# JuliaRobotics/RigidBodyDynamics.jl

Hardware: AMD Instinct MI355X
Metric: ABA dynamics! evals/sec (Atlas 30-DoF, batch) (higher is better)
Workload: dtype f64

## Files before the change

### rigidbodydynamics.jl_amd/csrc/rbd_bank.hpp

```cpp
#pragma once

#ifndef RBD_BANK_WAVES
#define RBD_BANK_WAVES 2
#endif
#ifndef RBD_BANK_FK_LDS
#define RBD_BANK_FK_LDS 0
#endif
#ifndef RBD_BANK_HANDOFF_LDS
#define RBD_BANK_HANDOFF_LDS 0
#endif

#ifdef RBD_BANK_FIXED_NL
#define RBD_BANK_UNROLL _Pragma("unroll")
namespace rbd { constexpr int kBankNs[] = {RBD_BANK_FIXED_NS}; }
#define RBD_BK_NL RBD_BANK_FIXED_NL
#define RBD_BK_L0 RBD_BANK_FIXED_L0
#define RBD_BK_NS(l) kBankNs[l]
#ifdef RBD_BANK_FIXED_PERM
#define RBD_BK_PERM(l) (((RBD_BANK_FIXED_PERM) >> (l)) & 1ull)
#else
#define RBD_BK_PERM(l) (kBankNs[l] > 1)
#endif
#else
#define RBD_BANK_UNROLL _Pragma("unroll 1")
#define RBD_BK_NL M.nlevels
#define RBD_BK_L0 M.L0
#define RBD_BK_NS(l) ns_next(nss, M.ns_desc)
#define RBD_BK_PERM(l) ((M.perm_down >> (l)) & 1)
#endif

namespace rbd {

template <typename T> struct alignas(2 * sizeof(T)) Pair2 { T a, b; };

RBD_DEV void wave_lds_sync() {
  __builtin_amdgcn_fence(__ATOMIC_RELEASE, "wavefront");
  __builtin_amdgcn_wave_barrier();
  __builtin_amdgcn_fence(__ATOMIC_ACQUIRE, "wavefront");
}


#define RBD_MASSIGN6(MOV)                                                                                                              \
  unsigned long long sv;                                                                                                               \
  asm volatile("s_and_saveexec_b64 %[sv], %[mk]\n\t" MOV " %[d0], %[s0]\n\t" MOV " %[d1], %[s1]\n\t" MOV " %[d2], %[s2]\n\t" MOV          \
               " %[d3], %[s3]\n\t" MOV " %[d4], %[s4]\n\t" MOV " %[d5], %[s5]\n\ts_mov_b64 exec, %[sv]\n\ts_nop 0"                         \
               : [sv] "=&s"(sv), [d0] "+v"(d[0]), [d1] "+v"(d[1]), [d2] "+v"(d[2]), [d3] "+v"(d[3]), [d4] "+v"(d[4]), [d5] "+v"(d[5])    \
               : [mk] "s"(mask), [s0] "v"(s[0]), [s1] "v"(s[1]), [s2] "v"(s[2]), [s3] "v"(s[3]), [s4] "v"(s[4]), [s5] "v"(s[5])          \
               : "scc")
RBD_DEV void massign6(unsigned long long mask, double* d, const double* s) { RBD_MASSIGN6("v_mov_b64"); }
RBD_DEV void massign6(unsigned long long mask, float* d, const float* s) { RBD_MASSIGN6("v_mov_b32"); }
template <typename T, int N> RBD_DEV void massign(bool m, T* d, const T* s) {
  static_assert(N % 6 == 0, "blocks of 6");
  const unsigned long long mask = __builtin_amdgcn_ballot_w64(m);
#pragma unroll
  for (int k = 0; k < N; k += 6) massign6(mask, d + k, s + k);
}

enum { PK_KIN = 0, PK_FWD = 6, PARK_PAIRS = 16, PK_XCH = 16, XCH_PAIRS = 14, BANK_LDS_PAIRS = PARK_PAIRS + XCH_PAIRS };

template <typename T, int N> RBD_DEV void lds_put(Pair2<T>* col, int pair0, const T* x) {
#pragma unroll
  for (int i = 0; i < (N + 1) / 2; ++i) {
    Pair2<T> v;
    v.a = x[2 * i];
    v.b = (2 * i + 1 < N) ? x[2 * i + 1] : T(0);
    col[(pair0 + i) * 256] = v;
  }
}
template <typename T, int N> RBD_DEV void lds_get(const Pair2<T>* col, int pair0, T* x) {
#pragma unroll
  for (int i = 0; i < (N + 1) / 2; ++i) {
    const Pair2<T> v = col[(pair0 + i) * 256];
    x[2 * i] = v.a;
    if (2 * i + 1 < N) x[2 * i + 1] = v.b;
  }
}

__host__ __device__ constexpr int sym_row(int e) { return e < 6 ? 0 : e < 11 ? 1 : e < 15 ? 2 : e < 18 ? 3 : e < 20 ? 4 : 5; }
__host__ __device__ constexpr int sym_col(int e) { return e - SI(sym_row(e), sym_row(e)) + sym_row(e); }

template <typename T> struct BankRegs {
  Body<T> b;
  const T* rb;
  int pcol;
  T K[24];
  RBD_DEV T* R() { return K; }
  RBD_DEV T* p() { return K + 9; }
  RBD_DEV T* Tw() { return K + 12; }
  RBD_DEV T* vJ() { return K + 18; }
  T S[6], cb[6], IA[21], pA[6], U[6], Dinv, u;
  T tj[6];
  T acc[6], vd[6];
};

template <typename T> RBD_DEV void load_bank_body(const BankModel& M, int k, long B, Body<T>& b) {
  const int tid = blockIdx.x * blockDim.x + threadIdx.x;
  b.lane = threadIdx.x & 63;
  const long wave = tid >> 6;
  const int lps = M.lps;
  b.sub = b.lane & (lps - 1);
  b.base = b.lane - b.sub;
  b.state = wave * (64 / lps) + (b.lane / lps);
  b.valid = (b.sub < M.nbk[k]) && (b.state < B);
  const int4* ib4 = reinterpret_cast<const int4*>(M.ib[k] + (b.sub < M.nbk[k] ? b.sub : 0) * IB_STRIDE);
  const int4 w0 = ib4[0], w1 = ib4[1], w2 = ib4[2], w3 = ib4[3];
  static_assert(IB_PARENT == 0 && IB_JTYPE == 1 && IB_QOFF == 2 && IB_VOFF == 3 && IB_LEVEL == 4 && IB_NCHILD == 5 && IB_ORIG == 6 && IB_CHILD0 == 7 &&
                IB_MAXCHILD == 8 && IB_FLAGS == 15 && IB_STRIDE == 16, "record layout");
  b.parent = w0.x; b.jtype = w0.y; b.qoff = w0.z; b.voff = w0.w;
  b.level = b.valid ? w1.x : -1;
  b.nchild = w1.y; b.orig = w1.z;
  b.child[0] = w1.w; b.child[1] = w2.x; b.child[2] = w2.y; b.child[3] = w2.z; b.child[4] = w2.w; b.child[5] = w3.x; b.child[6] = w3.y; b.child[7] = w3.z;
  b.flags = w3.w;
  b.plane = b.parent >= 0 ? b.base + b.parent : b.lane;
}

template <typename T, bool SIMPLE>
RBD_DEV void bank_fk_commit(bool mine, BankRegs<T>& c, const T* k18 , const T* XR, const T* Xp, const T* tl) {
  const T* pR = k18;
  const T* pp = k18 + 9;
  const T* pT = k18 + 12;
  T n[24];
  matmul3(pR, XR, n);
  matvec3(pR, Xp, n + 9);
#pragma unroll
  for (int k = 0; k < 3; ++k) n[9 + k] += pp[k];
  if (SIMPLE) {
    T S[6];
    matvec3(n, tl, S);
    cross3(n + 9, S, S + 3);
#pragma unroll
    for (int k = 0; k < 6; ++k) n[12 + k] = pT[k] + S[k] * tl[3];
    massign<T, 18>(mine, c.K, n);
  } else {
    xmotion(n, n + 9, tl, n + 18);
#pragma unroll
    for (int k = 0; k < 6; ++k) n[12 + k] = pT[k] + n[18 + k];
    massign<T, 24>(mine, c.K, n);
  }
}
template <typename T, bool SIMPLE> RBD_DEV void bank_fk_step(const BankModel& M, int l, bool perm, BankRegs<T>& c, Pair2<T>* lds, const T* XR, const T* Xp, const T* tl) {
  T k18[18];
// ... 55 lines not shown
    }
  }
  {
    T g[7], h[7];
    g[0] = gv.IA[20] - W[5] * gv.U[5];
    Iac[5] += g[0] * gv.cb[5];
#pragma unroll
    for (int k = 0; k < 6; ++k) g[1 + k] = gv.pA[k] + Iac[k] + W[k] * gv.u;
    if (MODE == 0) {
#pragma unroll
      for (int e = 0; e < 7; ++e) h[e] = from_next_lane(g[e]);
    }
    if (xw) lds_put<T, 7>(mycol, PK_XCH + 10, g);
    if (MODE == 0) {
      if (take0) {
        RBD_KEEP_BRANCH();
        tk.IA[20] += h[0];
#pragma unroll
        for (int k = 0; k < 6; ++k) tk.pA[k] += h[1 + k];
      }
    }
  }
  if (xw) {
    wave_lds_sync();
#pragma unroll 1
    for (int s = (MODE == 1 ? 0 : 1); s < ns; ++s) {
      if (takes && s < tk.b.nchild) {
        RBD_KEEP_BRANCH();
        const Pair2<T>* src = lds + (threadIdx.x - tk.b.sub + child_sel(tk.b, s));
        T x[28];
        lds_get<T, 28>(src, PK_XCH, x);
#pragma unroll
        for (int e = 0; e < 21; ++e) tk.IA[e] += x[e];
#pragma unroll
        for (int k = 0; k < 6; ++k) tk.pA[k] += x[21 + k];
      }
    }
    wave_lds_sync();
  }
}

template <typename T> RBD_DEV void bank_joint_accel(bool mine, BankRegs<T>& r, const T* a_parent) {
  T ap[6], n[6];
#pragma unroll
  for (int k = 0; k < 6; ++k) ap[k] = a_parent[k] + r.cb[k];
  const T x = r.Dinv * (r.u - dot6(r.U, ap));
#pragma unroll
  for (int k = 0; k < 6; ++k) n[k] = ap[k] + r.S[k] * x;
  massign<T, 6>(mine, r.acc, n);
  r.vd[0] = mine ? x : r.vd[0];
}
template <typename T> RBD_DEV void bank_accel_step(const BankModel& M, int l, bool perm, BankRegs<T>& c, Pair2<T>* lds) {
  T ap[6];
  if (RBD_BANK_FK_LDS || perm) {
    if (c.b.level == l - 1 && c.b.nchild >= 1) {
      RBD_KEEP_BRANCH();
      lds_put<T, 6>(lds + threadIdx.x, PK_XCH, c.acc);
    }
    wave_lds_sync();
    lds_get<T, 6>(lds + c.pcol, PK_XCH, ap);
    wave_lds_sync();
  } else {
#pragma unroll
    for (int k = 0; k < 6; ++k) ap[k] = from_prev_lane(c.acc[k]);
  }
  bank_joint_accel(c.b.level == l, c, ap);
}

#ifdef RBD_PROFILE_PHASES
__device__ long long rbd_bank_phase_clock[16];
#define RBD_MARK(i) do { if (blockIdx.x == 0 && threadIdx.x == 0) rbd_bank_phase_clock[i] = clock64(); } while (0)
#else
#define RBD_MARK(i)
#endif

template <typename T, bool R> struct InPtr { typedef const T* type; };
template <typename T> struct InPtr<T, true> { typedef const T* __restrict__ type; };

template <typename T, bool FUSED, bool SIMPLE>
RBD_DEV void aba_bank_body(const BankModel& M, long B, typename InPtr<T, !FUSED>::type q, typename InPtr<T, !FUSED>::type v, const T* __restrict__ tau,
                           const T* __restrict__ fext, T* __restrict__ vdot, T* __restrict__ qdot, Layout Lq, Layout Lv, Layout Lf, const MkFuse& F,
                           Pair2<T>* const lds) {
  Pair2<T>* const col = lds + threadIdx.x;
  RBD_MARK(0);
  BankRegs<T> r0, r1;
  auto fetch = [&](int k, BankRegs<T>& c, T* qj, T* vj) {
    load_bank_body(M, k, B, c.b);
    c.rb = reinterpret_cast<const T*>(M.rb[k]) + (c.b.sub < M.nbk[k] ? c.b.sub : 0) * RB_STRIDE;
    c.pcol = (int)threadIdx.x - c.b.sub + (c.b.parent >= 0 ? c.b.parent : c.b.sub);
    if (SIMPLE) {
      const bool fl = c.b.jtype == RBD_JOINT_QUAT_FLOATING;
      const long sc = c.b.state < B ? c.b.state : B - 1;
      const T* qp = q + ((long)c.b.qoff * Lq.sk + sc * Lq.sb);
      const long va = (long)c.b.voff * Lv.sk + sc * Lv.sb;
      const bool hv = v != nullptr, ht = tau != nullptr;
      qj[0] = qp[0];
      vj[0] = hv ? v[va] : T(0);
      c.tj[0] = ht ? tau[va] : T(0);
#pragma unroll
      for (int k2 = 1; k2 < 7; ++k2) qj[k2] = T(0);
#pragma unroll
      for (int k2 = 1; k2 < 6; ++k2) { vj[k2] = T(0); c.tj[k2] = T(0); }
      if (fl) {
        RBD_KEEP_BRANCH();
#pragma unroll
        for (int k2 = 1; k2 < 7; ++k2) qj[k2] = qp[k2 * Lq.sk];
        if (hv) {
#pragma unroll
          for (int k2 = 1; k2 < 6; ++k2) vj[k2] = v[va + k2 * Lv.sk];
        }
        if (ht) {
#pragma unroll
          for (int k2 = 1; k2 < 6; ++k2) c.tj[k2] = tau[va + k2 * Lv.sk];
        }
      }
    } else {
      load_joint_q(c.b, q, Lq, qj);
      load_joint_v(c.b, v, Lv, vj);
      load_joint_v(c.b, tau, Lv, c.tj);
    }
  };
  auto setup = [&](BankRegs<T>& c, T* qj, T* vj, T* XR, T* Xp, T* tl, T* ta ) {
    if (SIMPLE) {
      const bool fl = c.b.jtype == RBD_JOINT_QUAT_FLOATING;
      const T ax[3] = {c.rb[RB_AXIS], c.rb[RB_AXIS + 1], c.rb[RB_AXIS + 2]};
      T Rj[9], pj[3] = {T(0), T(0), T(0)};
      T sn, cs;
      ta[0] = ax[0]; ta[1] = ax[1]; ta[2] = ax[2]; ta[3] = vj[0];
      sincos_fast(qj[0], &sn, &cs);
      rot_axis_sc(ax, sn, cs, Rj);
#pragma unroll
      for (int k = 0; k < 3; ++k) { tl[k] = ax[k] * vj[0]; tl[3 + k] = T(0); }
      if (fl) {
        RBD_KEEP_BRANCH();
        rot_quat(qj[0], qj[1], qj[2], qj[3], Rj);
        pj[0] = qj[4]; pj[1] = qj[5]; pj[2] = qj[6];
#pragma unroll
        for (int k = 0; k < 6; ++k) tl[k] = vj[k];
        if (qdot != nullptr && c.b.valid) {
          const T w = qj[0], x = qj[1], y = qj[2], z = qj[3];
          T o[7];
          o[0] = (-x * vj[0] - y * vj[1] - z * vj[2]) * T(0.5);
          o[1] = (w * vj[0] - z * vj[1] + y * vj[2]) * T(0.5);
          o[2] = (z * vj[0] + w * vj[1] - x * vj[2]) * T(0.5);
          o[3] = (-y * vj[0] + x * vj[1] + w * vj[2]) * T(0.5);
          matvec3(Rj, vj + 3, o + 4);
#pragma unroll
          for (int k = 0; k < 7; ++k) qdot[(long)(c.b.qoff + k) * Lq.sk + c.b.state * Lq.sb] = o[k];
        }
      } else if (qdot != nullptr && c.b.valid) {
        qdot[(long)c.b.qoff * Lq.sk + c.b.state * Lq.sb] = vj[0];
      }
      T XpR[9], Xpp[3];
#pragma unroll
      for (int k = 0; k < 9; ++k) XpR[k] = c.rb[RB_XPR + k];
#pragma unroll
      for (int k = 0; k < 3; ++k) Xpp[k] = c.rb[RB_XPP + k];
      matmul3(XpR, Rj, XR);
      matvec3(XpR, pj, Xp);
#pragma unroll
      for (int k = 0; k < 3; ++k) Xp[k] += Xpp[k];
    } else {
      store_qdot(c.b, qdot, Lq, qj, vj);
      local_transform(c.b, c.rb, qj, XR, Xp);
      local_joint_motion(c.b, c.rb, vj, tl);
    }
#pragma unroll
    for (int i = 0; i < 9; ++i) c.R()[i] = XR[i];
#pragma unroll
    for (int i = 0; i < 3; ++i) c.p()[i] = Xp[i];
    xmotion(c.R(), c.p(), tl, c.Tw());
    if (SIMPLE) {
      c.K[18] = ta[3];
      c.K[19] = T(0);
    } else {
#pragma unroll
      for (int i = 0; i < 6; ++i) c.vJ()[i] = c.Tw()[i];
    }
  };
  auto terms = [&](BankRegs<T>& c, bool accumulate) {
    const bool floating = c.b.jtype == RBD_JOINT_QUAT_FLOATING;
    if (SIMPLE) {
      const T ax[3] = {c.rb[RB_AXIS], c.rb[RB_AXIS + 1], c.rb[RB_AXIS + 2]};
      matvec3(c.R(), ax, c.S);
      cross3(c.p(), c.S, c.S + 3);
    } else {
      T e1[6] = {T(1), T(0), T(0), T(0), T(0), T(0)}, sl[6];
      local_joint_motion(c.b, c.rb, e1, sl);
      xmotion(c.R(), c.p(), sl, c.S);
    }
    if (floating || (!SIMPLE && joint_nv(c.b.jtype) == 0)) {
#pragma unroll
      for (int i = 0; i < 6; ++i) c.S[i] = T(0);
    }
    if (SIMPLE) {
      se3_comm(c.Tw(), c.S, c.cb);
#pragma unroll
      for (int i = 0; i < 6; ++i) c.cb[i] *= c.K[18];
    } else {
      se3_comm(c.Tw(), c.vJ(), c.cb);
    }
    RInertia<T> I;
    T Jb[6], mc[3], fe[6];
#pragma unroll
    for (int i = 0; i < 6; ++i) Jb[i] = c.rb[RB_J + i];
#pragma unroll
    for (int i = 0; i < 3; ++i) mc[i] = c.rb[RB_MC + i];
    inertia_to_root(Jb, mc, c.rb[RB_M], c.R(), c.p(), I);
    T Io[21], po[6];
    sym6_from_inertia(I, Io);
    momentum_cross(I, c.Tw(), po);
    load_body_wrench(c.b, fext, Lf, fe);
#pragma unroll
    for (int i = 0; i < 21; ++i) c.IA[i] = accumulate ? c.IA[i] + Io[i] : Io[i];
#pragma unroll
    for (int i = 0; i < 6; ++i) c.pA[i] = accumulate ? c.pA[i] + (po[i] - fe[i]) : po[i] - fe[i];
#pragma unroll
    for (int i = 0; i < 6; ++i) c.U[i] = T(0);
    c.Dinv = T(0);
    c.u = T(0);
    if (floating) xforce(c.R(), c.p(), c.tj, c.U);
  };

  T qj0[7], vj0[6], qj1[7], vj1[6];
  fetch(0, r0, qj0, vj0);
  fetch(1, r1, qj1, vj1);
  if (FUSED) {
    if (F.close_prev) {
      mk_stage_lane(r0.b, 4, (T)F.dt, qj0, vj0, (const T*)nullptr, F.W, (T*)F.q_state, (T*)F.v_state, Lq, Lv);
      mk_stage_lane(r1.b, 4, (T)F.dt, qj1, vj1, (const T*)nullptr, F.W, (T*)F.q_state, (T*)F.v_state, Lq, Lv);
    }
    mk_stage_lane(r0.b, F.stage, (T)F.dt, qj0, vj0, (const T*)nullptr, F.W, (T*)F.q_state, (T*)F.v_state, Lq, Lv);
    mk_stage_lane(r1.b, F.stage, (T)F.dt, qj1, vj1, (const T*)nullptr, F.W, (T*)F.q_state, (T*)F.v_state, Lq, Lv);
    pd_control_lane(r0.b, F, Lq, qj0, vj0, r0.tj);
    pd_control_lane(r1.b, F, Lq, qj1, vj1, r1.tj);
  }
  {
    T XR[9], Xp[3], tl[6], ta[4];
    setup(r0, qj0, vj0, XR, Xp, tl, ta);
    RBD_MARK(1);
RBD_BANK_UNROLL
    for (int l = 1; l < RBD_BK_L0; ++l) bank_fk_step<T, SIMPLE>(M, l, RBD_BK_PERM(l), r0, lds, XR, Xp, SIMPLE ? ta : tl);
  }
  {
    T XR[9], Xp[3], tl[6], ta[4];
    RBD_MARK(2);
    setup(r1, qj1, vj1, XR, Xp, tl, ta);
    RBD_MARK(3);
    lds_put<T, (SIMPLE ? 20 : 24)>(col, PK_KIN, r0.K);
    wave_lds_sync();
    bank_fk_cross<T, SIMPLE>(RBD_BK_L0, r1, lds, XR, Xp, SIMPLE ? ta : tl);
RBD_BANK_UNROLL
    for (int l = RBD_BK_L0 + 1; l < RBD_BK_NL; ++l) bank_fk_step<T, SIMPLE>(M, l, RBD_BK_PERM(l), r1, lds, XR, Xp, SIMPLE ? ta : tl);
  }
  RBD_MARK(4);
  terms(r1, false);
  RBD_MARK(5);

  NsStream nss = ns_begin(M.ns_desc);
  (void)nss;
RBD_BANK_UNROLL
  for (int l = RBD_BK_NL - 1; l > RBD_BK_L0; --l) {
    bank_finish_joint<T, SIMPLE>(l, r1);
    bank_handoff<T, RBD_BANK_HANDOFF_LDS>(l, RBD_BK_NS(l), r1, r1, lds);
  }
  bank_finish_joint<T, SIMPLE>(RBD_BK_L0, r1);
  RBD_MARK(6);
#pragma unroll
  for (int i = 0; i < 21; ++i) r0.IA[i] = T(0);
#pragma unroll
  for (int i = 0; i < 6; ++i) r0.pA[i] = T(0);
  bank_handoff<T, 1>(RBD_BK_L0, RBD_BK_NS(RBD_BK_L0), r1, r0, lds);
  {
    lds_get<T, (SIMPLE ? 20 : 24)>(col, PK_KIN, r0.K);
    T f20[20];
#pragma unroll
    for (int i = 0; i < 6; ++i) { f20[i] = r1.U[i]; f20[8 + i] = r1.S[i]; f20[14 + i] = r1.cb[i]; }
    f20[6] = r1.Dinv;
    f20[7] = r1.u;
    lds_put<T, 20>(col, PK_FWD, f20);
  }
  RBD_MARK(7);
  terms(r0, true);
  RBD_MARK(8);
RBD_BANK_UNROLL
  for (int l = RBD_BK_L0 - 1; l >= 1; --l) {
    bank_finish_joint<T, SIMPLE>(l, r0);
    bank_handoff<T, RBD_BANK_HANDOFF_LDS>(l, RBD_BK_NS(l), r0, r0, lds);
  }
  bank_finish_joint<T, SIMPLE>(0, r0);
  RBD_MARK(9);

#pragma unroll
  for (int i = 0; i < 6; ++i) { r0.acc[i] = T(0); r0.vd[i] = T(0); }
  {
    const T a0[6] = {T(0), T(0), T(0), T(-M.gravity[0]), T(-M.gravity[1]), T(-M.gravity[2])};
    BankRegs<T>& c = r0;
    const bool fl0 = c.b.level == 0 && c.b.jtype == RBD_JOINT_QUAT_FLOATING;
    T fa[6] = {T(0), T(0), T(0), T(0), T(0), T(0)}, fv[6] = {T(0), T(0), T(0), T(0), T(0), T(0)};
    if (fl0) {
      RBD_KEEP_BRANCH();
      T rhs[6], d[6], k12[12];
#pragma unroll
      for (int i = 0; i < 6; ++i) rhs[i] = c.U[i] - c.pA[i];
      sym6_solve(c.IA, rhs, fa);
#pragma unroll
      for (int i = 0; i < 6; ++i) d[i] = fa[i] - a0[i];
      lds_get<T, 12>(col, PK_KIN, k12);
      xmotion_inv(k12, k12 + 9, d, fv);
    }
    massign<T, 6>(fl0, c.acc, fa);
    massign<T, 6>(fl0, c.vd, fv);
    bank_joint_accel(c.b.level == 0 && !fl0, c, a0);
  }
RBD_BANK_UNROLL
  for (int l = 1; l < RBD_BK_L0; ++l) bank_accel_step<T>(M, l, RBD_BK_PERM(l), r0, lds);
  RBD_MARK(10);
  if (vdot) store_joint_v(r0.b, vdot, Lv, r0.vd);
  if (FUSED) store_joint_v(r0.b, (T*)F.W.vd[F.stage], Lv, r0.vd);
  {
    T f20[20];
    lds_get<T, 20>(col, PK_FWD, f20);
#pragma unroll
    for (int i = 0; i < 6; ++i) {
      r1.U[i] = f20[i];
      r1.S[i] = f20[8 + i];
      r1.cb[i] = f20[14 + i];
      r1.acc[i] = T(0);
      r1.vd[i] = T(0);
    }
    r1.Dinv = f20[6];
    r1.u = f20[7];
  }
  {
    lds_put<T, 6>(col, PK_XCH, r0.acc);
    wave_lds_sync();
    T ap[6];
    lds_get<T, 6>(lds + r1.pcol, PK_XCH, ap);
    wave_lds_sync();
    bank_joint_accel(r1.b.level == RBD_BK_L0, r1, ap);
  }
RBD_BANK_UNROLL
  for (int l = RBD_BK_L0 + 1; l < RBD_BK_NL; ++l) bank_accel_step<T>(M, l, RBD_BK_PERM(l), r1, lds);
  RBD_MARK(11);
  if (vdot) store_joint_v(r1.b, vdot, Lv, r1.vd);
  if (FUSED) store_joint_v(r1.b, (T*)F.W.vd[F.stage], Lv, r1.vd);
}
#ifndef RBD_BANK_FIXED_NL
template <typename T, bool FUSED, bool SIMPLE>
__global__ __launch_bounds__(256, RBD_BANK_WAVES) void aba_bank_kernel(BankModel M, long B, typename InPtr<T, !FUSED>::type q, typename InPtr<T, !FUSED>::type v,
                                                         const T* __restrict__ tau, const T* __restrict__ fext, T* __restrict__ vdot,
                                                         T* __restrict__ qdot, Layout Lq, Layout Lv, Layout Lf, MkFuse F) {
  extern __shared__ double bank_lds_raw[];
  aba_bank_body<T, FUSED, SIMPLE>(M, B, q, v, tau, fext, vdot, qdot, Lq, Lv, Lf, F, reinterpret_cast<Pair2<T>*>(bank_lds_raw));
}
#endif

enum { RNEA_LDS_PAIRS = 12 };
template <typename T> struct RneaRegs {
  Body<T> b;
  const T* rb;
  int pcol;
  T K[24], w[6];
  RBD_DEV T* R() { return K; }
  RBD_DEV T* p() { return K + 9; }
  RBD_DEV T* Tw() { return K + 12; }
  RBD_DEV T* acc() { return K + 18; }
};

template <typename T, bool SIMPLE>
RBD_DEV void rnea_fk_commit(bool mine, RneaRegs<T>& c, const T* k24, const T* XR, const T* Xp, const T* tl, const T* al) {
  const T* pR = k24;
  const T* pp = k24 + 9;
  const T* pT = k24 + 12;
  const T* pa = k24 + 18;
  T n[24], vJ[6], nT[6], cr[6], aj[6];
  matmul3(pR, XR, n);
  matvec3(pR, Xp, n + 9);
#pragma unroll
  for (int k = 0; k < 3; ++k) n[9 + k] += pp[k];
  if (SIMPLE) {
    T S[6];
    matvec3(n, tl, S);
    cross3(n + 9, S, S + 3);
#pragma unroll
    for (int k = 0; k < 6; ++k) { vJ[k] = S[k] * tl[3]; aj[k] = S[k] * tl[4]; }
  } else {
    xmotion(n, n + 9, tl, vJ);
    xmotion(n, n + 9, al, aj);
  }
#pragma unroll
  for (int k = 0; k < 6; ++k) { n[12 + k] = pT[k] + vJ[k]; nT[k] = -n[12 + k]; }
  se3_comm(nT, pT, cr);
#pragma unroll
  for (int k = 0; k < 6; ++k) n[18 + k] = pa[k] + cr[k] + aj[k];
  massign<T, 24>(mine, c.K, n);
}
template <typename T, bool SIMPLE>
RBD_DEV void rnea_fk_step(const BankModel& M, int l, bool perm, RneaRegs<T>& c, Pair2<T>* lds, const T* XR, const T* Xp, const T* tl, const T* al) {
  T k24[24];
  if (perm) {
    if (c.b.level == l - 1 && c.b.nchild >= 1) {
      RBD_KEEP_BRANCH();
      lds_put<T, 24>(lds + threadIdx.x, 0, c.K);
    }
    wave_lds_sync();
    lds_get<T, 24>(lds + c.pcol, 0, k24);
    wave_lds_sync();
  } else {
#pragma unroll
    for (int k = 0; k < 24; ++k) k24[k] = from_prev_lane(c.K[k]);
  }
  rnea_fk_commit<T, SIMPLE>(c.b.level == l, c, k24, XR, Xp, tl, al);
}

template <typename T, bool CROSS> RBD_DEV void rnea_gather(int l, int ns, const RneaRegs<T>& gv, RneaRegs<T>& tk) {
  const bool takes = (tk.b.level == l - 1);
  if (!CROSS) {
    T t[6];
#pragma unroll
    for (int k = 0; k < 6; ++k) t[k] = from_next_lane(gv.w[k]);
    if (takes && tk.b.nchild >= 1) {
      RBD_KEEP_BRANCH();
#pragma unroll
      for (int k = 0; k < 6; ++k) tk.w[k] += t[k];
    }
  }
// ... 197 lines not shown
```

### rigidbodydynamics.jl_amd/csrc/rbd_capi.hip

```cpp
#include "rbd_capi_internal.hpp"
enum { BANK_LDS_PAIRS_HOST = 30 };

thread_local std::string g_last_hip_error;

static int joint_nq_host(int t) {
  switch (t) {
    case RBD_JOINT_FIXED: return 0;
    case RBD_JOINT_REVOLUTE: case RBD_JOINT_PRISMATIC: return 1;
    case RBD_JOINT_QUAT_FLOATING: return 7;
    case RBD_JOINT_PLANAR: return 3;
    case RBD_JOINT_QUAT_SPHERICAL: return 4;
    case RBD_JOINT_SINCOS_REVOLUTE: return 2;
    default: return -1;
  }
}
static int joint_nv_host(int t) {
  switch (t) {
    case RBD_JOINT_FIXED: return 0;
    case RBD_JOINT_REVOLUTE: case RBD_JOINT_PRISMATIC: case RBD_JOINT_SINCOS_REVOLUTE: return 1;
    case RBD_JOINT_QUAT_FLOATING: return 6;
    case RBD_JOINT_PLANAR: case RBD_JOINT_QUAT_SPHERICAL: return 3;
    default: return -1;
  }
}

long tune(const char* key, long dflt, bool* has) {
  if (has) *has = false;
  const char* e = getenv("RBD_TUNE");
  if (!e) return dflt;
  const size_t n = strlen(key);
  for (const char* p = e; *p;) {
    const char* end = strchr(p, ',');
    const size_t len = end ? (size_t)(end - p) : strlen(p);
    if (len > n && memcmp(p, key, n) == 0 && p[n] == '=') { if (has) *has = true; return atol(p + n + 1); }
    if (len == n && memcmp(p, key, n) == 0) { if (has) *has = true; return 1; }
    if (!end) break;
    p = end + 1;
  }
  return dflt;
}

static std::string loop_program_source(const rbd_model* m, int dtype, std::vector<int32_t>* xi_store);
static int bank_simple(const rbd_model* m);
static std::string bank_program_source(const rbd_model* m, int dtype, int simple);
static std::string walk_program_source(const rbd_model* m, int dtype, bool rerooted, int kind = 0, int pair = 0);
static bool walk_program_rerooted(const rbd_model* m, int dtype, int pair = 0);

extern "C" {

int rbd_version(void) { return RBD_HIP_H_VERSION; }
static std::string program_source(const rbd_model* m, int32_t dtype, int32_t family) {
  if (!m || (dtype != RBD_F32 && dtype != RBD_F64) || family < 0 || family > SPEC_KIN) return std::string();
  if (family == SPEC_KIN) return m->spec_plan().ok ? spec_source(m->spec_plan(), m->nb, m->nq, m->nv, m->row_mask.data(), m->gravity, dtype, SPEC_KIN) : std::string();
  if (family == SPEC_FAMILIES + 6) return walk_program_source(m, dtype, walk_program_rerooted(m, dtype), 2);
  if (family == SPEC_FAMILIES + 7) return dtype == RBD_F32 ? walk_program_source(m, dtype, walk_program_rerooted(m, dtype, 1), 2, 1) : std::string();
  std::vector<int32_t> xi;
  if (family < SPEC_FAMILIES && !m->spec_plan().ok) return std::string();
  if (family == SPEC_FAMILIES + 5) return bank_program_source(m, dtype, bank_simple(m));
  return family == SPEC_FAMILIES + 4 ? (dtype == RBD_F32 ? walk_program_source(m, dtype, false, 1, 1) : std::string())
         : family == SPEC_FAMILIES + 3 ? (dtype == RBD_F32 ? walk_program_source(m, dtype, walk_program_rerooted(m, dtype, 1), 0, 1) : std::string())
         : family == SPEC_FAMILIES + 2 ? walk_program_source(m, dtype, false, 1)
         : family == SPEC_FAMILIES + 1 ? walk_program_source(m, dtype, walk_program_rerooted(m, dtype))
         : family == SPEC_FAMILIES ? loop_program_source(m, dtype, &xi)
                                   : spec_source(m->spec_plan(), m->nb, m->nq, m->nv, m->row_mask.data(), m->gravity, dtype, family);
}
static bool family_is_walk(int family) { return (family > SPEC_FAMILIES && family <= SPEC_FAMILIES + 4) || family == SPEC_FAMILIES + 6 || family == SPEC_FAMILIES + 7; }
static int code_object_get(const std::string& src, bool walk, bool wait, std::vector<char>* code, std::string* log) {
  return walk ? jit_walk_code_object_get(src, wait, code, log) : jit_code_object_get(src, wait, code, log);
}
int64_t rbd_jit_source(const rbd_model_t* m, int32_t dtype, int32_t family, char* buf, int64_t cap) {
  const std::string s = program_source(m, dtype, family);
  if (s.empty()) return -1;
  if (buf && cap > 0) { const int64_t n = std::min<int64_t>(cap - 1, (int64_t)s.size()); memcpy(buf, s.data(), (size_t)n); buf[n] = 0; }
  return (int64_t)s.size();
}
void rbd_jit_wait_idle(void) { jit_wait_idle(); }
int rbd_jit_check_walk_object(const char* source, const void* code, int64_t size, char* log, int64_t cap) {
  if (log && cap > 0) log[0] = 0;
  if (!source || !code || size <= 0) return RBD_ERR_INVALID_ARGUMENT;
  std::vector<char> c((const char*)code, (const char*)code + size);
  std::string l;
  const bool ok = jit_walk_admit(source, &c, &l);
  if (log && cap > 0) { const int64_t n = std::min<int64_t>(cap - 1, (int64_t)l.size()); memcpy(log, l.data(), (size_t)n); log[n] = 0; }
  return ok ? RBD_OK : RBD_ERR_UNSUPPORTED;
}
int rbd_jit_status(const rbd_model_t* m, int32_t dtype, int32_t family) {
  const std::string src = program_source(m, dtype, family);
  if (src.empty() || !jit_available()) return -1;
  std::vector<char> code;
  std::string log;
  const int js = code_object_get(src, family_is_walk(family), false, &code, &log);
  return js == JIT_READY ? 1 : js == JIT_PENDING ? 0 : -1;
}
int rbd_jit_precompile(const rbd_model_t* m, int32_t dtype, char* log, int64_t cap) {
  if (log && cap > 0) log[0] = 0;
  if (!m || (dtype != RBD_F32 && dtype != RBD_F64)) return RBD_ERR_INVALID_ARGUMENT;
  if ((!m->spec_plan().ok && !m->loop_fused_ok && !(m->track.ok && m->walk.ok) && m->bank_lps <= 0) || !jit_available()) return RBD_ERR_UNSUPPORTED;
  struct Job { std::string src; bool walk; int family; int state; double seconds; std::string log; };
  std::vector<Job> jobs;
  for (int family : {4, 9, 5, 6, 10, 7, 8, 0, 1, 2, 11, 3})
    jobs.push_back({program_source(m, dtype, family), family_is_walk(family), family, JIT_PENDING, 0.0, std::string()});
  int part = 0, parts = 1;
  if (const char* e = getenv("RBD_JIT_PRECOMPILE_PART")) { if (sscanf(e, "%d/%d", &part, &parts) != 2 || parts < 1 || part < 0 || part >= parts) { part = 0; parts = 1; } }
  int idx = 0;
  for (Job& j : jobs) {
    if (j.src.empty()) { j.state = -1; continue; }
    if (idx++ % parts != part) j.state = -1;
  }
  const auto t0 = std::chrono::steady_clock::now();
  int st = RBD_OK;
  for (bool pending = true; pending;) {
    pending = false;
    for (Job& j : jobs) {
      if (j.state != JIT_PENDING) continue;
      std::vector<char> code;
      j.state = code_object_get(j.src, j.walk, false, &code, &j.log);
      if (j.state == JIT_PENDING) pending = true;
      else j.seconds = std::chrono::duration<double>(std::chrono::steady_clock::now() - t0).count();
    }
    if (pending) usleep(20000);
  }
  std::string all;
  for (const Job& j : jobs) {
    if (j.state < 0) continue;
    char b[160];
    snprintf(b, sizeof b, "[rbd_jit] family %d (%s): %s after %.1f s\n", j.family, dtype == RBD_F64 ? "f64" : "f32", j.state == JIT_READY ? "ready" : j.walk ? "not used" : "FAILED", j.seconds);
    all += b;
    all += j.log;
    if (j.state == JIT_FAILED && !j.walk) st = RBD_ERR_HIP;
  }
  if (log && cap > 0) { const int64_t n = std::min<int64_t>(cap - 1, (int64_t)all.size()); memcpy(log, all.data(), (size_t)n); log[n] = 0; }
  return st;
}

const char* rbd_status_string(int s) {
  switch (s) {
    case RBD_OK: return "ok";
    case RBD_ERR_INVALID_ARGUMENT: return "invalid argument";
    case RBD_ERR_DIMENSION_MISMATCH: return "dimension mismatch";
    case RBD_ERR_UNSUPPORTED: return "unsupported joint type or feature";
    case RBD_ERR_NO_DEVICE: return "no HIP device available (librbd_hip has no CPU fallback)";
    case RBD_ERR_HIP: return "HIP runtime error";
    case RBD_ERR_OUT_OF_MEMORY: return "out of memory";
    case RBD_ERR_HAS_LOOPS: return "This method can currently only handle tree Mechanisms.";
    case RBD_ERR_NOT_POSITIVE_DEFINITE: return "mass matrix not positive definite";
    default: return "unknown status";
  }
}
const char* rbd_last_hip_error(void) { return g_last_hip_error.c_str(); }

static int build_loop_tables(rbd_model* m, const rbd_flat_model_t* d) {
  const int nb = m->nb;
  for (int l = 0; l < d->n_loops; ++l) {
    const rbd_loop_joint_t& lj = d->loops[l];
    const int nvl = joint_nv_host(lj.joint_type);
    if (nvl < 0) return RBD_ERR_INVALID_ARGUMENT;
    if (lj.predecessor >= nb || lj.successor >= nb || lj.predecessor < -1 || lj.successor < -1) return RBD_ERR_INVALID_ARGUMENT;
    const int ncl = 6 - nvl;
    double Tl[36] = {0};
    const double* R = lj.rotation_from_z_aligned;
    if (lj.joint_type == RBD_JOINT_REVOLUTE || lj.joint_type == RBD_JOINT_SINCOS_REVOLUTE) {
      for (int r = 0; r < 3; ++r) { Tl[0 + r] = R[3 * r]; Tl[6 + r] = R[3 * r + 1]; Tl[12 + 3 + r] = R[3 * r]; Tl[18 + 3 + r] = R[3 * r + 1]; Tl[24 + 3 + r] = R[3 * r + 2]; }
    } else if (lj.joint_type == RBD_JOINT_PRISMATIC) {
      for (int r = 0; r < 3; ++r) { Tl[0 + r] = R[3 * r]; Tl[6 + r] = R[3 * r + 1]; Tl[12 + r] = R[3 * r + 2]; Tl[18 + 3 + r] = R[3 * r]; Tl[24 + 3 + r] = R[3 * r + 1]; }
    } else if (lj.joint_type == RBD_JOINT_FIXED) {
      for (int c = 0; c < 6; ++c) Tl[6 * c + c] = 1;
    } else if (lj.joint_type == RBD_JOINT_QUAT_SPHERICAL) {
      for (int c = 0; c < 3; ++c) Tl[6 * c + 3 + c] = 1;
    } else if (lj.joint_type == RBD_JOINT_PLANAR) {
      for (int r = 0; r < 3; ++r) { Tl[0 + 3 + r] = R[3 * r + 2]; Tl[6 + r] = R[3 * r]; Tl[12 + r] = R[3 * r + 1]; }
    } else if (lj.joint_type != RBD_JOINT_QUAT_FLOATING) {
      return RBD_ERR_UNSUPPORTED;
    }
    const int path_begin = (int)m->loop_path.size() / 2;
    int a = lj.predecessor, b = lj.successor;
    while (a != b) {
      if (a > b) { m->loop_path.push_back(a); m->loop_path.push_back(-1); a = d->parent[a]; }
      else { m->loop_path.push_back(b); m->loop_path.push_back(1); b = d->parent[b]; }
    }
    const int path_end = (int)m->loop_path.size() / 2;
    const int32_t rec[8] = {lj.predecessor, lj.successor, lj.joint_type, m->nc, ncl, path_begin, path_end, 0};
    m->loop_i.insert(m->loop_i.end(), rec, rec + 8);
    double r64[64] = {0};
// ... 116 lines not shown
  m->ib.assign((size_t)nb * IB_STRIDE, -1);
  for (int s = 0; s < nb; ++s) {
    const int i = m->order[s];
    const int p = d->parent[i];
    const int ps = p < 0 ? -1 : m->slot_of[p];
    level[s] = ps < 0 ? 0 : level[ps] + 1;
    if (level[s] + 1 > m->nlevels) m->nlevels = level[s] + 1;
    int32_t* ib = &m->ib[(size_t)s * IB_STRIDE];
    ib[IB_PARENT] = ps; ib[IB_JTYPE] = d->joint_type[i]; ib[IB_QOFF] = d->q_offset[i]; ib[IB_VOFF] = d->v_offset[i];
    ib[IB_LEVEL] = level[s]; ib[IB_ORIG] = i; ib[IB_FLAGS] = 0;
    if (d->joint_type[i] == RBD_JOINT_QUAT_FLOATING && ps >= 0) m->inner_floating = 1;
    const int nc = (int)kids[i].size();
    if (nc > IB_MAXCHILD) { delete m; return RBD_ERR_UNSUPPORTED; }
    ib[IB_NCHILD] = nc;
    for (int k = 0; k < nc; ++k) ib[IB_CHILD0 + k] = m->slot_of[kids[i][k]];
    if (nc > m->maxchild) m->maxchild = nc;
  }
  for (int s = 0; s < nb; ++s) {
    const int i = m->order[s];
    for (int k = 0; k < (int)kids[i].size(); ++k) m->ib[(size_t)s * IB_STRIDE + IB_CHILD0 + k] = m->slot_of[kids[i][k]];
  }
  if (m->nlevels > MAX_LEVELS) { delete m; return RBD_ERR_UNSUPPORTED; }
  m->nslots.assign(MAX_LEVELS, 0);
  m->perm_down = 0;
  for (int s = 0; s < nb; ++s) {
    const int nc = m->ib[(size_t)s * IB_STRIDE + IB_NCHILD];
    if (nc > 0 && nc > m->nslots[level[s] + 1]) m->nslots[level[s] + 1] = nc;
    const int ps = m->ib[(size_t)s * IB_STRIDE + IB_PARENT];
    if (ps >= 0 && ps != s - 1) m->perm_down |= (uint64_t)1 << level[s];
    if (ps >= 0 && m->ib[(size_t)ps * IB_STRIDE + IB_CHILD0] != ps + 1) { delete m; return RBD_ERR_INVALID_ARGUMENT; }
  }
  m->rb.assign((size_t)nb * RB_STRIDE, 0.0);
  for (int s = 0; s < nb; ++s) {
    const int i = m->order[s];
    double* rb = &m->rb[(size_t)s * RB_STRIDE];
    for (int k = 0; k < 3; ++k) rb[RB_AXIS + k] = d->joint_axis[3 * i + k];
    if (d->joint_axis2) for (int k = 0; k < 3; ++k) rb[RB_AXIS2 + k] = d->joint_axis2[3 * i + k];
    for (int k = 0; k < 9; ++k) rb[RB_XPR + k] = d->pred_rot[9 * i + k];
    for (int k = 0; k < 3; ++k) rb[RB_XPP + k] = d->pred_trans[3 * i + k];
    const double* J = d->inertia_moment + 9 * i;
    rb[RB_J + 0] = J[0]; rb[RB_J + 1] = J[1]; rb[RB_J + 2] = J[2]; rb[RB_J + 3] = J[4]; rb[RB_J + 4] = J[5]; rb[RB_J + 5] = J[8];
    for (int k = 0; k < 3; ++k) rb[RB_MC + k] = d->inertia_cross[3 * i + k];
    rb[RB_M] = d->inertia_mass[i];
  }
  m->dof_body.assign(m->nv > 0 ? m->nv : 1, 0);
  for (int i = 0; i < nb; ++i)
    for (int k = 0; k < joint_nv_host(d->joint_type[i]); ++k) m->dof_body[d->v_offset[i] + k] = m->slot_of[i];
  m->anc.assign((size_t)nb * m->nlevels, -1);
  for (int s = 0; s < nb; ++s) {
    int a = s;
    for (int k = 0; k < m->nlevels && a >= 0; ++k) { m->anc[(size_t)s * m->nlevels + k] = a; a = m->ib[(size_t)a * IB_STRIDE + IB_PARENT]; }
  }
  m->row_words = std::max(1, (m->nv + 63) / 64);
  m->row_mask.assign((size_t)(m->nv > 0 ? m->nv : 1) * m->row_words, 0);
  for (int r = 0; r < m->nv; ++r) {
    const int sr = m->dof_body[r];
    for (int c = 0; c <= r; ++c) {
      const int sc = m->dof_body[c];
      bool sup = false;
      for (int k = 0; k < m->nlevels; ++k) sup |= (m->anc[(size_t)sr * m->nlevels + k] == sc);
      if (sup) m->row_mask[(size_t)r * m->row_words + c / 64] |= (uint64_t)1 << (c % 64);
    }
  }
  m->nc = 0;
  m->jt_ref.assign(d->joint_type, d->joint_type + nb);
  m->parent_ref.assign(d->parent, d->parent + nb);
  m->voff_ref.assign(d->v_offset, d->v_offset + nb);
  m->qoff_ref.assign(d->q_offset, d->q_offset + nb);
  for (int i = 0; i < nb; ++i) {
    const int jt = d->joint_type[i];
    if (jt == RBD_JOINT_QUAT_FLOATING) { m->mkf.push_back(d->q_offset[i]); m->mkf.push_back(d->v_offset[i]); }
    else if (jt == RBD_JOINT_REVOLUTE || jt == RBD_JOINT_PRISMATIC || jt == RBD_JOINT_SINCOS_REVOLUTE) { m->mk1.push_back(d->q_offset[i]); m->mk1.push_back(d->v_offset[i]); m->mk1.push_back(jt); }
  }
  m->loop_fused_ok = d->n_loops > 0 && nb <= 4 && m->nv <= 4;
  for (int i = 0; i < nb && m->loop_fused_ok; ++i) {
    const int t = d->joint_type[i];
    m->loop_fused_ok = d->parent[i] < i && (t == RBD_JOINT_REVOLUTE || t == RBD_JOINT_PRISMATIC || t == RBD_JOINT_SINCOS_REVOLUTE || t == RBD_JOINT_FIXED);
  }
  m->axis_ref.assign(d->joint_axis, d->joint_axis + 3 * nb);
  if (d->joint_axis2) m->axis2_ref.assign(d->joint_axis2, d->joint_axis2 + 3 * nb); else m->axis2_ref.assign(3 * nb, 0.0);
  if (int lst = build_loop_tables(m, d)) { delete m; return lst; }
  m->bank_aba_ok = (m->nloops == 0 && !m->has3dof && !m->inner_floating);
  if (m->nlevels >= 2) {
    std::vector<int> per_level(m->nlevels, 0);
    for (int s = 0; s < nb; ++s) per_level[level[s]]++;
    int best_L0 = 0, best_lanes = 1 << 30, best_diff = 1 << 30;
    for (int L0 = 1; L0 < m->nlevels; ++L0) {
      int cA = 0, cB = 0;
      for (int l = 0; l < m->nlevels; ++l) (l < L0 ? cA : cB) += per_level[l];
      int lanes = 1;
      while (lanes < std::max(cA, cB)) lanes <<= 1;
      const int diff = std::abs(cA - cB);
      if (lanes < best_lanes || (lanes == best_lanes && diff < best_diff)) { best_lanes = lanes; best_L0 = L0; best_diff = diff; }
    }
    if (best_lanes < m->lps) {
      m->bank_lps = best_lanes; m->bank_L0 = best_L0;
      std::vector<int> bslot(nb, -1);
      int cnt[2] = {0, 0};
      for (int s = 0; s < nb; ++s) bslot[s] = cnt[level[s] >= best_L0]++;
      m->bank_nb[0] = cnt[0]; m->bank_nb[1] = cnt[1];
      for (int k = 0; k < 2; ++k) { m->bank_ib[k].assign((size_t)std::max(cnt[k], 1) * IB_STRIDE, -1); m->bank_rb[k].assign((size_t)std::max(cnt[k], 1) * RB_STRIDE, 0.0); }
      m->bank_perm_down = 0;
      for (int s = 0; s < nb; ++s) {
        const int k = level[s] >= best_L0, j = bslot[s];
        const int32_t* src = &m->ib[(size_t)s * IB_STRIDE];
        int32_t* dst = &m->bank_ib[k][(size_t)j * IB_STRIDE];
        memcpy(dst, src, sizeof(int32_t) * IB_STRIDE);
        const int ps = src[IB_PARENT];
        dst[IB_PARENT] = ps < 0 ? -1 : bslot[ps];
        for (int c2 = 0; c2 < src[IB_NCHILD]; ++c2) dst[IB_CHILD0 + c2] = bslot[src[IB_CHILD0 + c2]];
        if (ps >= 0 && level[s] != best_L0 && bslot[ps] != j - 1) { m->bank_perm_down |= (uint64_t)1 << level[s]; dst[IB_FLAGS] |= BFD_NOTFIRST; }
        memcpy(&m->bank_rb[k][(size_t)j * RB_STRIDE], &m->rb[(size_t)s * RB_STRIDE], sizeof(double) * RB_STRIDE);
      }
    }
  }
  {
    int nheads = 0;
    for (int s = 0; s < nb; ++s) {
      const int ps = m->ib[(size_t)s * IB_STRIDE + IB_PARENT];
      if (ps < 0 || m->ib[(size_t)ps * IB_STRIDE + IB_CHILD0] != s) ++nheads;
    }
    int G = 1;
    while (G < nheads && G < 4) G <<= 1;
    if (m->nloops == 0) m->chain = build_chain_plan(nb, m->ib, G);
    if (m->nloops == 0 && G <= 4) m->track = build_track_plan(nb, m->ib, m->rb, G);
    if (m->track.ok) m->walk = build_walk_plan(m->track.ns, m->track.G, m->track.ri);
    if (m->nloops == 0 && m->nv <= 64) m->state = build_state_plan(nb, m->ib, m->rb);
    if (m->nloops == 0 && m->nv <= 64 && !m->state.ok) m->state_wide = build_state_plan(nb, m->ib, m->rb, true);
  }
  if (m->bank_aba_ok) {
    m->rr = build_reroot(d);
    if (m->rr.ok) {
      const Reroot& R = m->rr;
      rbd_model::RrSlots& S = m->rrs;
      std::vector<std::vector<int>> kd(nb);
      for (int i = 0; i < nb; ++i) if (R.parent[i] >= 0) kd[R.parent[i]].push_back(i);
      std::vector<int> ord, slot(nb, -1), lev(nb, 0);
      {
        std::vector<int> stack{R.root};
        while (!stack.empty()) {
          const int i = stack.back(); stack.pop_back();
          slot[i] = (int)ord.size();
          ord.push_back(i);
          for (auto it = kd[i].rbegin(); it != kd[i].rend(); ++it) stack.push_back(*it);
        }
      }
      bool fits = (int)ord.size() == nb;
      for (int i = 0; i < nb && fits; ++i) fits = (int)kd[i].size() <= IB_MAXCHILD;
      if (fits) {
        S.ib.assign((size_t)nb * IB_STRIDE, -1);
        S.rb.assign((size_t)nb * RB_STRIDE, 0.0);
        S.nslots.assign(MAX_LEVELS, 0);
        for (int s2 = 0; s2 < nb; ++s2) {
          const int i = ord[s2], p = R.parent[i], ps = p < 0 ? -1 : slot[p];
          lev[s2] = ps < 0 ? 0 : lev[ps] + 1;
          if (lev[s2] + 1 > S.nlevels) S.nlevels = lev[s2] + 1;
          int32_t* ib = &S.ib[(size_t)s2 * IB_STRIDE];
          ib[IB_PARENT] = ps; ib[IB_JTYPE] = R.jtype[i]; ib[IB_QOFF] = R.qoff[i]; ib[IB_VOFF] = R.voff[i]; ib[IB_LEVEL] = lev[s2]; ib[IB_ORIG] = i;
          ib[IB_FLAGS] = R.flags[i];
          ib[IB_NCHILD] = (int)kd[i].size();
          for (int k = 0; k < (int)kd[i].size(); ++k) ib[IB_CHILD0 + k] = slot[kd[i][k]];
          double* rb = &S.rb[(size_t)s2 * RB_STRIDE];
          for (int k = 0; k < 3; ++k) { rb[RB_AXIS + k] = R.axis[3 * i + k]; rb[RB_AXIS2 + k] = R.axis2[3 * i + k]; rb[RB_XPP + k] = R.Xpp[3 * i + k]; rb[RB_MC + k] = R.mc[3 * i + k]; }
          for (int k = 0; k < 9; ++k) rb[RB_XPR + k] = R.XpR[9 * i + k];
          for (int k = 0; k < 6; ++k) rb[RB_J + k] = R.J6[6 * i + k];
          rb[RB_M] = R.mass[i];
        }
        for (int s2 = 0; s2 < nb; ++s2) {
          const int nc = S.ib[(size_t)s2 * IB_STRIDE + IB_NCHILD];
          if (nc > 0 && nc > S.nslots[lev[s2] + 1]) S.nslots[lev[s2] + 1] = nc;
        }
        int nheads = 0;
        for (int s2 = 0; s2 < nb; ++s2) {
          const int ps = S.ib[(size_t)s2 * IB_STRIDE + IB_PARENT];
          if (ps < 0 || S.ib[(size_t)ps * IB_STRIDE + IB_CHILD0] != s2) ++nheads;
        }
        int G = 1;
        while (G < nheads && G < 4) G <<= 1;
        S.track = build_track_plan(nb, S.ib, S.rb, G);
        if (S.track.ok) {
          S.walk = build_walk_plan(S.track.ns, S.track.G, S.track.ri);
          if (S.walk.ok)
            for (size_t k = 0; k < S.walk.wk.size(); ++k) {
              const int e = S.track.tab[k];
              if (e >= 0) S.walk.wk[k] |= S.ib[(size_t)e * IB_STRIDE + IB_FLAGS] << 8;
            }
        }
        S.ok = true;
      }
    }
  }
  *out = m;
  return RBD_OK;
}

int rbd_model_destroy(rbd_model_t* m) {
  delete m;
  return RBD_OK;
}

int rbd_model_bank_plan(const rbd_model_t* m, int32_t* lanes, int32_t* first_level_of_bank1, int32_t* bodies_bank0, int32_t* bodies_bank1,
                        int32_t* aba_in_scope) {
  if (!m) return RBD_ERR_INVALID_ARGUMENT;
  if (m->bank_lps <= 0) return RBD_ERR_UNSUPPORTED;
  if (lanes) *lanes = m->bank_lps;
  if (first_level_of_bank1) *first_level_of_bank1 = m->bank_L0;
  if (bodies_bank0) *bodies_bank0 = m->bank_nb[0];
  if (bodies_bank1) *bodies_bank1 = m->bank_nb[1];
  if (aba_in_scope) *aba_in_scope = m->bank_aba_ok;
  return RBD_OK;
}

int rbd_model_chain_plan(const rbd_model_t* m, int32_t* tracks, int32_t* steps, int32_t* lds_fields, int32_t* table, int32_t capacity) {
  if (!m) return RBD_ERR_INVALID_ARGUMENT;
  if (!m->chain.ok) return RBD_ERR_UNSUPPORTED;
  if (tracks) *tracks = m->chain.G;
  if (steps) *steps = m->chain.ns;
  if (lds_fields) *lds_fields = 0;
  if (table) {
    if (capacity < (int32_t)m->chain.tab.size()) return RBD_ERR_DIMENSION_MISMATCH;
    for (size_t i = 0; i < m->chain.tab.size(); ++i) table[i] = m->chain.tab[i] < 0 ? -1 : m->order[m->chain.tab[i]];
  }
  return RBD_OK;
}

int rbd_model_track_plan(const rbd_model_t* m, int32_t* dims, int32_t* table, int32_t table_cap, int32_t* ri, int32_t ri_cap, double* rr, int32_t rr_cap) {
  if (!m) return RBD_ERR_INVALID_ARGUMENT;
  if (!m->track.ok) return RBD_ERR_UNSUPPORTED;
  const TrackPlan& P = m->track;
  if (dims) { dims[0] = P.G; dims[1] = P.ns; dims[2] = P.nA; dims[3] = P.nB; dims[4] = P.has_floating; dims[5] = P.general; }
  if (table) {
    if (table_cap < (int32_t)P.tab.size()) return RBD_ERR_DIMENSION_MISMATCH;
    for (size_t i = 0; i < P.tab.size(); ++i) table[i] = P.tab[i] < 0 ? -1 : m->order[P.tab[i]];
  }
  if (ri) {
    if (ri_cap < (int32_t)(P.ri.size() + P.sf.size())) return RBD_ERR_DIMENSION_MISMATCH;
    memcpy(ri, P.ri.data(), P.ri.size() * sizeof(int32_t));
    memcpy(ri + P.ri.size(), P.sf.data(), P.sf.size() * sizeof(int32_t));
  }
  if (rr) { if (rr_cap < (int32_t)P.rr.size()) return RBD_ERR_DIMENSION_MISMATCH; memcpy(rr, P.rr.data(), P.rr.size() * sizeof(double)); }
  return RBD_OK;
}

int rbd_model_reroot_plan(const rbd_model_t* m, int32_t* dims, int32_t* ri, int32_t ri_cap, double* rr, int32_t rr_cap, int32_t* wk, int32_t wk_cap,
                          int32_t* chain_i, double* chain_r, double* fxp) {
  if (!m) return RBD_ERR_INVALID_ARGUMENT;
  if (!m->rrs.ok || !m->rrs.track.ok || !m->rrs.walk.ok) return RBD_ERR_UNSUPPORTED;
  const TrackPlan& P = m->rrs.track;
  const Reroot& R = m->rr;
  const int nch = (int)(R.chain_i.size() / RC_I_STRIDE);
  if (dims) {
    const int32_t d[12] = {P.G, P.ns, P.nA, P.nB, P.has_floating, P.general, m->rrs.walk.nS, nch, R.fq, R.fv, R.root, R.fb};
    memcpy(dims, d, sizeof d);
  }
  if (ri) {
    if (ri_cap < (int32_t)(P.ri.size() + P.sf.size())) return RBD_ERR_DIMENSION_MISMATCH;
    memcpy(ri, P.ri.data(), P.ri.size() * sizeof(int32_t));
    memcpy(ri + P.ri.size(), P.sf.data(), P.sf.size() * sizeof(int32_t));
  }
  if (rr) { if (rr_cap < (int32_t)P.rr.size()) return RBD_ERR_DIMENSION_MISMATCH; memcpy(rr, P.rr.data(), P.rr.size() * sizeof(double)); }
  if (wk) { if (wk_cap < (int32_t)m->rrs.walk.wk.size()) return RBD_ERR_DIMENSION_MISMATCH; memcpy(wk, m->rrs.walk.wk.data(), m->rrs.walk.wk.size() * sizeof(int32_t)); }
  if (chain_i) memcpy(chain_i, R.chain_i.data(), R.chain_i.size() * sizeof(int32_t));
  if (chain_r) memcpy(chain_r, R.chain_r.data(), R.chain_r.size() * sizeof(double));
  if (fxp) memcpy(fxp, R.fXp, sizeof R.fXp);
  return RBD_OK;
}

int rbd_model_dims(const rbd_model_t* m, int32_t* nb, int32_t* nq, int32_t* nv, int32_t* nc) {
  if (!m) return RBD_ERR_INVALID_ARGUMENT;
  if (nb) *nb = m->nb;
// ... 43 lines not shown
  }
  if (device < 0 || device >= ndev) return RBD_ERR_INVALID_ARGUMENT;
  HIP_TRY(hipSetDevice(device));
  std::unique_ptr<rbd_ws> owner(new (std::nothrow) rbd_ws());
  rbd_ws* w = owner.get();
  if (!w) return RBD_ERR_OUT_OF_MEMORY;
  w->model = m; w->device = device; w->dtype = dtype; w->max_batch = max_batch; w->stream = (hipStream_t)stream;
  if (m->big) {
    int st = upload(w->d_big_tbl, m->big_tbl.data(), m->big_tbl.size() * sizeof(int32_t));
    if (st == RBD_OK) st = upload_real(w->d_big_rb, m->big_rb, dtype);
    if (st == RBD_OK) { int zero = 0; st = upload(w->d_notpd, &zero, sizeof(int)); }
    if (st == RBD_OK) st = upload_loop_tables(w, m, dtype);
    if (st == RBD_OK) st = upload_contact_tables(w, m, dtype);
    if (st != RBD_OK) return st;
    w->big.nb = m->nb; w->big.nq = m->nq; w->big.nv = m->nv; w->big.tbl = (const int32_t*)w->d_big_tbl.p; w->big.rb = w->d_big_rb.p;
    memcpy(w->big.gravity, m->gravity, sizeof w->big.gravity);
    w->last_kernel = "big_* kernels (one thread per state, HBM scratch)";
    *out = owner.release();
    return RBD_OK;
  }
  int st = upload(w->d_ib, m->ib.data(), m->ib.size() * sizeof(int32_t));
  if (st == RBD_OK) st = upload_real(w->d_rb, m->rb, dtype);
  if (st == RBD_OK) st = upload(w->d_dof_body, m->dof_body.data(), m->dof_body.size() * sizeof(int32_t));
  if (st == RBD_OK) st = upload(w->d_anc, m->anc.data(), m->anc.size() * sizeof(int32_t));
  if (st == RBD_OK) st = upload(w->d_row_mask, m->row_mask.data(), m->row_mask.size() * sizeof(uint64_t));
  if (st == RBD_OK) { int zero = 0; st = upload(w->d_notpd, &zero, sizeof(int)); }
  if (st == RBD_OK) st = upload_loop_tables(w, m, dtype);
  if (st != RBD_OK) return st;
  DevModel& dm = w->dm;
  dm.nb = m->nb; dm.nq = m->nq; dm.nv = m->nv; dm.lps = m->lps; dm.nlevels = m->nlevels; dm.maxchild = m->maxchild; dm.maxnvj = m->maxnvj;
  dm.ib = (const int32_t*)w->d_ib.p; dm.rb = w->d_rb.p;
  dm.perm_down = m->perm_down;
  dm.inner_floating = m->inner_floating;
  dm.has3dof = m->has3dof;
  dm.nheavy = 0;
  for (int s2 = 0; s2 < m->nb; ++s2) {
    const int jt = m->ib[(size_t)s2 * IB_STRIDE + IB_JTYPE];
    if (jt != RBD_JOINT_QUAT_FLOATING && jt != RBD_JOINT_QUAT_SPHERICAL) continue;
    if (dm.nheavy < 4) { dm.heavy[dm.nheavy][0] = jt; dm.heavy[dm.nheavy][1] = m->ib[(size_t)s2 * IB_STRIDE + IB_QOFF]; dm.heavy[dm.nheavy][2] = m->ib[(size_t)s2 * IB_STRIDE + IB_VOFF]; }
    ++dm.nheavy;
  }
  nslots_pack_desc(dm.ns_desc, m->nslots.data(), m->nlevels);
  dm.dof_body = (const int32_t*)w->d_dof_body.p; dm.anc = (const int32_t*)w->d_anc.p; dm.row_mask = (const uint64_t*)w->d_row_mask.p; dm.row_words = m->row_words;
  memcpy(dm.gravity, m->gravity, sizeof dm.gravity);
  if (m->bank_lps > 0) {
    BankModel& bm = w->bm;
    for (int k = 0; k < 2 && st == RBD_OK; ++k) {
      st = upload(w->d_bank_ib[k], m->bank_ib[k].data(), m->bank_ib[k].size() * sizeof(int32_t));
      if (st != RBD_OK) break;
      st = upload_real(w->d_bank_rb[k], m->bank_rb[k], dtype);
      bm.ib[k] = (const int32_t*)w->d_bank_ib[k].p; bm.rb[k] = w->d_bank_rb[k].p; bm.nbk[k] = m->bank_nb[k];
    }
    if (st != RBD_OK) return st;
    bm.lps = m->bank_lps; bm.nlevels = m->nlevels; bm.L0 = m->bank_L0; bm.perm_down = m->bank_perm_down;
    bm.simple = bank_simple(m);
    if (tune("bank_generic", 0)) bm.simple = 0;
    nslots_pack_desc(bm.ns_desc, m->nslots.data(), m->nlevels);
    memcpy(bm.gravity, m->gravity, sizeof bm.gravity);
    w->bank_min_batch = 0;
    w->rnea_bank_min_batch = 0;
    {
      int ncu = 256;
      (void)hipDeviceGetAttribute(&ncu, hipDeviceAttributeMultiprocessorCount, device);
      if (m->has3dof) w->rnea_bank_min_batch = (long)ncu * 28 + 1;
    }
    { bool has; const long t = tune("bank_min_batch", 0, &has); if (has) w->bank_min_batch = w->rnea_bank_min_batch = t; }
    {
      int ncu = 256;
      (void)hipDeviceGetAttribute(&ncu, hipDeviceAttributeMultiprocessorCount, device);
      const size_t lds = (size_t)BANK_LDS_PAIRS_HOST * 256 * 2 * (dtype == RBD_F64 ? 8 : 4);
      const long per_cu = std::max<long>(1, std::min<long>(2, (long)(160 * 1024 / lds)));
      w->bank_resident_states = (long)ncu * per_cu * (256 / m->bank_lps);
    }
  }
  if (m->rrs.ok) {
    const Reroot& R = m->rr;
    const rbd_model::RrSlots& S = m->rrs;
    st = upload(w->d_rr_chain_i, R.chain_i.data(), R.chain_i.size() * sizeof(int32_t));
    if (st == RBD_OK) st = upload_real(w->d_rr_chain_r, R.chain_r, dtype);
    RerootView V{};
    V.nchain = (int32_t)(R.chain_i.size() / RC_I_STRIDE); V.fq = R.fq; V.fv = R.fv;
    V.chain_i = (const int32_t*)w->d_rr_chain_i.p; V.chain_r = w->d_rr_chain_r.p;
    memcpy(V.fXp, R.fXp, sizeof V.fXp);
    if (st == RBD_OK && S.track.ok && S.walk.ok) {
      const TrackPlan& P = S.track;
      st = upload(w->d_rrtrack_ri, P.ri.data(), P.ri.size() * sizeof(int32_t));
      if (st == RBD_OK) st = upload_real(w->d_rrtrack_rr, P.rr, dtype);
      if (st == RBD_OK) st = upload(w->d_rrwalk_wk, S.walk.wk.data(), S.walk.wk.size() * sizeof(int32_t));
      WalkModel& wm = w->wm_rr;
      wm.ns = P.ns; wm.G = P.G; wm.nA = P.nA; wm.nB = P.nB; wm.nS = S.walk.nS; wm.nq = m->nq; wm.nv = m->nv; wm.reroot = V;
      wm.ri = (const int32_t*)w->d_rrtrack_ri.p; wm.rr = w->d_rrtrack_rr.p; wm.wk = (const int32_t*)w->d_rrwalk_wk.p;
      for (int k = 0; k < 5; ++k) { wm.sfm[k] = 0; for (int s2 = 0; s2 < P.ns; ++s2) wm.sfm[k] |= (uint64_t)((P.sf[s2] >> k) & 1) << s2; }
      memcpy(wm.gravity, m->gravity, sizeof wm.gravity);
      const size_t es2 = dtype == RBD_F64 ? 8 : 4;
      w->walk_rr_lds_bytes = walk_lds_bytes(P.ns, P.G, m->nq, m->nv, P.nA, P.nB, S.walk.nS, es2, es2);
      if (w->walk_rr_lds_bytes > 160 * 1024) w->walk_rr_lds_bytes = 0;
      w->walk_rr_lds_bytes_pair = dtype == RBD_F32 ? walk_lds_bytes(P.ns, P.G, m->nq, m->nv, P.nA, P.nB, S.walk.nS, 8, 4) : 0;
      if (w->walk_rr_lds_bytes_pair > 160 * 1024) w->walk_rr_lds_bytes_pair = 0;
      w->walk_rr = st == RBD_OK && (w->walk_rr_lds_bytes > 0 || w->walk_rr_lds_bytes_pair > 0);
    }
    if (st != RBD_OK) return st;
  }
  if (m->track.ok) {
    const TrackPlan& P = m->track;
    st = upload(w->d_track_ri, P.ri.data(), P.ri.size() * sizeof(int32_t));
    if (st == RBD_OK) st = upload_real(w->d_track_rr, P.rr, dtype);
    if (st != RBD_OK) return st;
    TrackModel& tm = w->tm;
    tm.ns = P.ns; tm.G = P.G; tm.nA = P.nA; tm.nB = P.nB; tm.ri = (const int32_t*)w->d_track_ri.p; tm.rr = w->d_track_rr.p;
    for (int k = 0; k < 5; ++k) { tm.sfm[k] = 0; for (int s2 = 0; s2 < P.ns; ++s2) tm.sfm[k] |= (uint64_t)((P.sf[s2] >> k) & 1) << s2; }
    memcpy(tm.gravity, m->gravity, sizeof tm.gravity);
  }
  if ((st = upload_contact_tables(w, m, dtype)) != RBD_OK) return st;
  if (m->track.ok && m->walk.ok) {
    const TrackPlan& P = m->track;
    st = upload(w->d_walk_wk, m->walk.wk.data(), m->walk.wk.size() * sizeof(int32_t));
    if (st != RBD_OK) return st;
    w->spec_walk_min_batch = 8192;
    { bool has; const long t = tune("spec_walk_min_batch", 0, &has); if (has) w->spec_walk_min_batch = t; }
    w->spec_walk_f32 = tune("spec_walk_f32", 1) != 0;
    WalkModel& wm = w->wm;
    wm.ns = P.ns; wm.G = P.G; wm.nA = P.nA; wm.nB = P.nB; wm.nS = m->walk.nS; wm.nq = m->nq; wm.nv = m->nv;
    wm.ri = (const int32_t*)w->d_track_ri.p; wm.rr = w->d_track_rr.p; wm.wk = (const int32_t*)w->d_walk_wk.p;
    for (int k = 0; k < 5; ++k) wm.sfm[k] = w->tm.sfm[k];
    memcpy(wm.gravity, m->gravity, sizeof wm.gravity);
    const size_t es = dtype == RBD_F64 ? 8 : 4;
    w->walk_lds_bytes = walk_lds_bytes(P.ns, P.G, m->nq, m->nv, P.nA, P.nB, m->walk.nS, es, es);
    if (w->walk_lds_bytes > 160 * 1024) w->walk_lds_bytes = 0;
    w->walk_lds_bytes_pair = dtype == RBD_F32 ? walk_lds_bytes(P.ns, P.G, m->nq, m->nv, P.nA, P.nB, m->walk.nS, 8, 4) : 0;
    if (w->walk_lds_bytes_pair > 160 * 1024) w->walk_lds_bytes_pair = 0;
    {
      const size_t l1 = std::max(w->walk_lds_bytes, w->walk_rr ? w->walk_rr_lds_bytes : (size_t)0), l2 = std::max(w->walk_lds_bytes_pair, w->walk_rr ? w->walk_rr_lds_bytes_pair : (size_t)0);
      const hipError_t e = by_dtype(dtype, [&](auto t) { return configure_walk_kernel<decltype(t)>(P.has_floating, P.general, l1, l2); });
      if (e != hipSuccess) { g_last_hip_error = std::string("configure_walk_kernel: ") + hipGetErrorString(e); return RBD_ERR_HIP; }
    }
    {
      int ncu = 256;
      (void)hipDeviceGetAttribute(&ncu, hipDeviceAttributeMultiprocessorCount, device);
      w->walk_pair_min_batch = (long)ncu * 64 + 1;
      { bool has; const long t = tune("walk_pair_min_batch", 0, &has); if (has) w->walk_pair_min_batch = t; }
    }
    {
      int ncu = 256;
      (void)hipDeviceGetAttribute(&ncu, hipDeviceAttributeMultiprocessorCount, device);
      w->walk_min_batch = (m->bank_lps > 0 && m->bank_aba_ok ? w->bank_resident_states : (long)ncu * 4 * 2 * (64 / m->lps)) + 1;
      const bool banked = m->bank_lps > 0 && m->bank_aba_ok;
      w->walk_one_round_batch = banked ? (long)ncu * (256 / m->bank_lps) + 1 : w->walk_min_batch;
      w->rnea_walk_min_batch = banked ? std::max<long>(w->walk_min_batch, (long)ncu * 2 * (256 / m->bank_lps) + 1) : w->walk_min_batch;
      if (bool has = false; (void)tune("spec_walk_min_batch", 0, &has), !has) w->spec_walk_min_batch = std::min<long>(w->spec_walk_min_batch, w->walk_one_round_batch);
    }
    { bool has; const long t = tune("walk_min_batch", 0, &has); if (has) w->walk_min_batch = t; }
  }
  if (m->state.ok && m->state.nlevels <= state_max_levels(dtype == RBD_F64 ? 8 : 4)) {
    const StatePlan& P = m->state;
    st = upload(w->d_state_ops, P.ops.data(), P.ops.size() * sizeof(int32_t));
    if (st == RBD_OK) st = upload(w->d_state_cols, P.cols.data(), P.cols.size() * sizeof(int32_t));
    if (st == RBD_OK) st = upload_real(w->d_state_sr, P.sr, dtype);
    if (st != RBD_OK) return st;
    StateModel& sm = w->sm;
    sm.nb = m->nb; sm.nq = m->nq; sm.nv = m->nv; sm.nops = P.nops; sm.nlevels = P.nlevels;
    sm.ops = (const int32_t*)w->d_state_ops.p; sm.cols = (const int32_t*)w->d_state_cols.p; sm.sr = w->d_state_sr.p; sm.row_mask = (const uint64_t*)w->d_row_mask.p;
    memcpy(sm.gravity, m->gravity, sizeof sm.gravity);
    int ncu = 256;
    (void)hipDeviceGetAttribute(&ncu, hipDeviceAttributeMultiprocessorCount, device);
    w->state_min_batch = (long)ncu * 4 * 64 / 2;
    { bool has; const long t = tune("state_min_batch", 0, &has); if (has) w->state_min_batch = t; }
// ... 79 lines not shown
  w->loop_gains = want;
  w->custom_gains = custom;
  return RBD_OK;
}

int rbd_workspace_bind_result(rbd_ws_t* w, void* M, void* c) {
  if (!w) return RBD_ERR_INVALID_ARGUMENT;
  for (void* p : {M, c}) {
    if (!p) continue;
    hipPointerAttribute_t a{};
    if (hipPointerGetAttributes(&a, p) != hipSuccess) { (void)hipGetLastError(); return RBD_ERR_INVALID_ARGUMENT; }
    if (a.type != hipMemoryTypeDevice && a.type != hipMemoryTypeManaged && a.type != hipMemoryTypeUnified) return RBD_ERR_INVALID_ARGUMENT;
  }
  w->bound_M = M;
  w->bound_c = c;
  return RBD_OK;
}

int rbd_sync(rbd_ws_t* w) {
  if (!w) return RBD_ERR_INVALID_ARGUMENT;
  HIP_TRY(hipSetDevice(w->device));
  HIP_TRY(hipStreamSynchronize(w->stream));
  int flag = 0;
  HIP_TRY(hipMemcpy(&flag, (int*)w->d_notpd.p, sizeof(int), hipMemcpyDeviceToHost));
  if (flag) {
    HIP_TRY(hipMemset((int*)w->d_notpd.p, 0, sizeof(int)));
    return RBD_ERR_NOT_POSITIVE_DEFINITE;
  }
  return RBD_OK;
}

int rbd_workspace_enable_timing(rbd_ws_t* w, int32_t enable) {
  if (!w) return RBD_ERR_INVALID_ARGUMENT;
  HIP_TRY(hipSetDevice(w->device));
  if (enable && !w->ev0) {
    HIP_TRY(hipEventCreate(&w->ev0));
    HIP_TRY(hipEventCreate(&w->ev1));
  }
  w->timing = enable ? 1 : 0;
  return RBD_OK;
}

const char* rbd_workspace_last_kernel(const rbd_ws_t* w) { return w ? w->last_kernel : ""; }

int rbd_workspace_last_kernel_ms(rbd_ws_t* w, float* ms) {
  if (!w || !ms || !w->ev_pending) return RBD_ERR_INVALID_ARGUMENT;
  HIP_TRY(hipEventSynchronize(w->ev1));
  HIP_TRY(hipEventElapsedTime(ms, w->ev0, w->ev1));
  return RBD_OK;
}

}

int ensure(DevBuf& b, size_t need) {
  if (b.bytes >= need) return RBD_OK;
  b.reset();
  HIP_TRY(hipMalloc(&b.p, need));
  b.bytes = need;
  return RBD_OK;
}

int upload(DevBuf& dst, const void* src, size_t bytes) {
  dst.reset();
  if (int st = ensure(dst, bytes ? bytes : 16)) return st;
  if (bytes) HIP_TRY(hipMemcpy(dst.p, src, bytes, hipMemcpyHostToDevice));
  return RBD_OK;
}

int upload_real(DevBuf& dst, const std::vector<double>& src, int dtype) {
  if (dtype == RBD_F64) return upload(dst, src.data(), src.size() * sizeof(double));
  const std::vector<float> f(src.begin(), src.end());
  return upload(dst, f.data(), f.size() * sizeof(float));
}

static int bank_simple(const rbd_model* m) {
  for (int i = 0; i < m->nb; ++i)
    if (m->jt_ref[i] != RBD_JOINT_REVOLUTE && !(m->jt_ref[i] == RBD_JOINT_QUAT_FLOATING && m->parent_ref[i] < 0)) return 0;
  return 1;
}
static std::string bank_program_source(const rbd_model* m, int dtype, int simple) {
  if (m->bank_lps <= 0) return std::string();
  return spec_bank_source(m->nlevels, m->bank_L0, m->nslots.data(), (unsigned long long)m->bank_perm_down, simple, dtype);
}
static std::string loop_program_source(const rbd_model* m, int dtype, std::vector<int32_t>* xi_store) {
  if (!m->loop_fused_ok) return std::string();
  xi_store->assign(3 * (size_t)m->nb, 0);
  for (int i = 0; i < m->nb; ++i) { (*xi_store)[3 * i] = m->parent_ref[i]; (*xi_store)[3 * i + 1] = m->qoff_ref[i]; (*xi_store)[3 * i + 2] = m->slot_of[i]; }
  LoopTables L{m->nb, m->nq, m->nv, m->nc, m->nloops, &m->loop_i, &m->loop_path, &m->jt_ref, &m->voff_ref, xi_store, &m->loop_r, &m->axis_ref, &m->axis2_ref, &m->rb, m->gravity};
  return spec_loop_source(L, dtype);
}
static bool walk_tables(const rbd_model* m, bool rerooted, WalkTables* W) {
  const TrackPlan* P; const WalkPlan* K;
  if (rerooted) { if (!m->rrs.ok || !m->rrs.track.ok || !m->rrs.walk.ok) return false; P = &m->rrs.track; K = &m->rrs.walk; }
  else { if (!m->track.ok || !m->walk.ok) return false; P = &m->track; K = &m->walk; }
  *W = WalkTables{};
  W->ns = P->ns; W->G = P->G; W->nA = P->nA; W->nB = P->nB; W->nS = K->nS; W->nq = m->nq; W->nv = m->nv; W->flt = P->has_floating; W->gen = P->general; W->rr = rerooted;
  W->ri = &P->ri; W->wk = &K->wk; W->rrc = &P->rr;
  W->mk1 = &m->mk1; W->mkf = &m->mkf;
  for (int k = 0; k < 5; ++k) { W->sfm[k] = 0; for (int s2 = 0; s2 < P->ns; ++s2) W->sfm[k] |= (uint64_t)((P->sf[s2] >> k) & 1) << s2; }
  if (rerooted) {
    W->nchain = (int)(m->rr.chain_i.size() / RC_I_STRIDE); W->fq = m->rr.fq; W->fv = m->rr.fv; W->chain_i = &m->rr.chain_i; W->chain_r = &m->rr.chain_r; W->fXp = m->rr.fXp;
    if (W->nchain < 1) return false;
  }
  return true;
}
static bool walk_program_rerooted(const rbd_model* m, int dtype, int pair) {
  WalkTables W;
  return tune("walk_no_reroot", 0) == 0 && walk_tables(m, true, &W) && walk_lds_bytes(W.ns, W.G, W.nq, W.nv, W.nA, W.nB, W.nS, (dtype == RBD_F64 || pair) ? 8 : 4, dtype == RBD_F64 ? 8 : 4) <= 160 * 1024;
}
static std::string walk_program_source(const rbd_model* m, int dtype, bool rerooted, int kind, int pair) {
  WalkTables W;
  if (!walk_tables(m, rerooted, &W)) return std::string();
  return walk_spec_source(W, dtype, kind, pair);
}
static bool capturing(rbd_ws* w);
template <class Source>
static hipModule_t spec_module(rbd_ws* w, SpecSlot& p, Source source, bool walk, bool wait, const char* fallback) {
  if (p.tried) return nullptr;
  if (!jit_available()) { p.tried = true; return nullptr; }
  if (capturing(w)) return nullptr;
  if (p.src.empty()) p.src = source();
  if (p.src.empty()) { p.tried = true; return nullptr; }
  std::string log;
  std::vector<char> code;
  const int js = code_object_get(p.src, walk, wait, &code, &log);
  if (js == JIT_PENDING) return nullptr;
  p.tried = true;
  std::string src;
  src.swap(p.src);
  if (js == JIT_FAILED || code.empty()) { g_last_hip_error = std::string("run-time compilation failed (") + fallback + "): " + log; return nullptr; }
  if (hipModuleLoadData(&p.mod, code.data()) != hipSuccess) { (void)hipGetLastError(); p.mod = nullptr; jit_cache_discard(src); return nullptr; }
  return p.mod;
}
static const int kNoScratchCheck = INT_MAX;
static hipFunction_t spec_kernel(hipModule_t mod, const char* name, int max_scratch, int* scratch = nullptr) {
  hipFunction_t f = nullptr;
  int bytes = 0;
  if (hipModuleGetFunction(&f, mod, name) != hipSuccess) { (void)hipGetLastError(); f = nullptr; }
  else if (max_scratch != kNoScratchCheck && (hipFuncGetAttribute(&bytes, HIP_FUNC_ATTRIBUTE_LOCAL_SIZE_BYTES, f) != hipSuccess || bytes > max_scratch)) { (void)hipGetLastError(); f = nullptr; }
  if (scratch) *scratch = bytes;
  return f;
}
static hipFunction_t spec_walk(rbd_ws* w, bool rerooted, int kind = 0, int pair = 0) {
  const int k = 4 * kind + (rerooted ? 2 : 0) + (pair ? 1 : 0);
  if (hipModule_t mod = spec_module(w, w->spec_prog[SPEC_WALK + k], [&] { return walk_program_source(w->model, w->dtype, rerooted, kind, pair); }, true, !jit_async(),
                                    "the interpreting kernel is used")) {
    const std::string name = std::string(kind == 1 ? "rnea_walk_spec_" : kind == 2 ? "aba_walk_sim_spec_" : "aba_walk_spec_") + walk_spec_suffix(w->dtype, pair);
    w->spec_walk[k].f = spec_kernel(mod, name.c_str(), w->spec_max_scratch);
  }
  return w->spec_walk[k].f;
}
int big_scratch(rbd_ws* w, int32_t B) { return ensure(w->d_big_scratch, esize(w) * big_scratch_elems(w->big, B)); }
static hipFunction_t spec_loop(rbd_ws* w) {
  auto source = [&] { std::vector<int32_t> xi; return loop_program_source(w->model, w->dtype, &xi); };
  if (hipModule_t mod = spec_module(w, w->spec_prog[SPEC_LOOP], source, false, !jit_async(), "the generic loop kernels are used"))
    w->spec_loop = spec_kernel(mod, w->dtype == RBD_F64 ? "loop_spec_f64" : "loop_spec_f32", 0);
  return w->spec_loop;
}

static bool spec_bank(rbd_ws* w) {
  SpecSlot& p = w->spec_prog[SPEC_BANK];
  if (w->model->bank_lps <= 0) p.tried = true;
  if (hipModule_t mod = spec_module(w, p, [&] { return bank_program_source(w->model, w->dtype, w->bm.simple); }, false, !jit_async(),
                                    "the banked kernels built with the library are used")) {
    const std::string sfx = w->dtype == RBD_F64 ? "f64" : "f32";
    w->spec_bank_aba.f = spec_kernel(mod, ("aba_bank_spec_" + sfx).c_str(), w->spec_max_scratch);
    w->spec_bank_fused = spec_kernel(mod, ("aba_bank_fused_spec_" + sfx).c_str(), w->spec_max_scratch);
    w->spec_bank_rnea.f = spec_kernel(mod, ("rnea_bank_spec_" + sfx).c_str(), w->spec_max_scratch);
  }
  return w->spec_bank_aba.f != nullptr;
}

namespace {
template <typename T>
int dynamics_loops_t(rbd_ws* w, int32_t B, const Opts& o, const void* dq, const void* dv, const void* dtau, const void* df, void* dvd, void* dqd,
                     void* dlam) {
  const rbd_model* m = w->model;
  const size_t es = sizeof(T);
  const int nv = m->nv, nc = m->nc;
  const long stride = (long)nv * nv + 2L * nc * nv + 2L * nc * nc + 2L * nv + 2L * nc;
  int st;
  if ((st = ensure(w->d_M, es * (size_t)nv * nv * B)) || (st = ensure(w->d_c, es * (size_t)nv * B)) ||
      (st = ensure(w->d_K, es * (size_t)(nc * nv > 0 ? nc * nv : 1) * B)) || (st = ensure(w->d_k, es * (size_t)(nc > 0 ? nc : 1) * B)) ||
      (st = ensure(w->d_body, es * (size_t)m->nb * 24 * B)) || (st = ensure(w->d_scratch, es * (size_t)stride * B)))
    return st;
  w->result_layout = o.layout; w->result_B = B;
  const Layout Lq = layout_of(o.layout, m->nq, B), Lv = layout_of(o.layout, nv, B), Lf = layout_of(o.layout, 6L * m->nb, B);
  const Layout Lm = layout_of(o.layout, (long)nv * nv, B), Lc = layout_of(o.layout, nc, B), Lk = layout_of(o.layout, (long)nc * nv, B);
  LoopView<T> V;
  V.nloops = m->nloops; V.nc = nc; V.nv = nv; V.nb = m->nb;
  V.li = (const int32_t*)w->d_loop_i.p; V.lr = (const T*)w->d_loop_r.p; V.path = (const int32_t*)w->d_loop_path.p;
  V.jt = (const int32_t*)w->d_jt_ref.p; V.voff = (const int32_t*)w->d_voff_ref.p; V.axis = (const T*)w->d_axis_ref.p; V.axis2 = (const T*)w->d_axis2_ref.p;
  V.xi = (const int32_t*)w->d_fused_i.p; V.rb = (const T*)w->d_rb.p;
  Timed t(w);
  const bool no_fused = w->loop_no_fused;
  if (hipFunction_t f = (m->loop_fused_ok && !no_fused) ? spec_loop(w) : nullptr) {
    long Bl = B;
    int stab = o.stabilization;
    void* dM = w->d_M.p; void* dc = w->d_c.p; void* dK = w->d_K.p; void* dk = w->d_k.p; int* notpd = (int*)w->d_notpd.p;
    Layout a_Lq = Lq, a_Lm = Lm, a_Lv = Lv, a_Lf = Lf, a_Lc = Lc, a_Lk = Lk;
    const T* gains = w->custom_gains ? (const T*)w->d_loop_r.p + 24 : nullptr;
    void* args[] = {&Bl, &stab, &dq, &dv, &dtau, &df, &dM, &dc, &dvd, &dqd, &dlam, &dK, &dk, &a_Lq, &a_Lm, &a_Lv, &a_Lf, &a_Lc, &a_Lk, &notpd, &gains};
    HIP_TRY(hipModuleLaunchKernel(f, (unsigned)((B + 63) / 64), 1, 1, 64, 1, 1, 0, w->stream, args, nullptr));
    w->last_kernel = "loop_spec (compiled for the mechanism at run time)";
    return RBD_OK;
  }
  if (m->loop_fused_ok && !no_fused &&
      launch_loop_fused<T>(V, B, o.stabilization, dq, dv, dtau, df, w->d_body.p, w->d_M.p, w->d_c.p, dvd, dqd, dlam, w->d_K.p, w->d_k.p, Lq, Lm, Lv, Lf, Lc, Lk, m->gravity,
                           (int*)w->d_notpd.p, w->stream)) {
    HIP_TRY(hipGetLastError());
    w->last_kernel = "loop_fused_small_kernel";
    return RBD_OK;
  }
  if (m->big) {
    if ((st = big_scratch(w, B))) return st;
    HIP_TRY(launch_big_rnea<T>(w->big, B, dq, dv, nullptr, df, w->d_c.p, dqd, w->d_big_scratch.p, nullptr, nullptr, Lq, Lv, Lf, w->stream));
    HIP_TRY(launch_big_export_body<T>(w->big, B, w->d_big_scratch.p, w->d_body.p, w->stream));
    HIP_TRY(launch_big_crba<T>(w->big, B, dq, w->d_M.p, w->d_big_scratch.p, Lq, Lm, w->stream));
    HIP_TRY(launch_loop_solve<T>(V, B, o.stabilization, w->d_body.p, w->d_M.p, w->d_c.p, dtau, dvd, dlam, w->d_K.p, w->d_k.p, w->d_scratch.p, stride, Lm, Lv, Lc, Lk,
                                 m->gravity, (int*)w->d_notpd.p, w->stream));
    w->last_kernel = "big_rnea + big_crba + loop_solve kernel";
    return RBD_OK;
  }
  HIP_TRY(launch_rnea<T>(w->dm, B, dq, dv, nullptr, df, w->d_c.p, dqd, w->d_body.p, Lq, Lv, Lf, w->stream));
  HIP_TRY(launch_crba<T>(w->dm, B, dq, w->d_M.p, Lq, Lm, 1, w->stream));
  HIP_TRY(launch_loop_solve<T>(V, B, o.stabilization, w->d_body.p, w->d_M.p, w->d_c.p, dtau, dvd, dlam, w->d_K.p, w->d_k.p, w->d_scratch.p, stride, Lm, Lv, Lc, Lk,
                               m->gravity, (int*)w->d_notpd.p, w->stream));
  w->last_kernel = "rnea_kernel + crba_kernel + loop_solve kernel";
  return RBD_OK;
}
int dynamics_loops(rbd_ws* w, int32_t B, const Opts& o, const void* dq, const void* dv, const void* dtau, const void* df, void* dvd, void* dqd, void* dlam) {
  return by_dtype(w->dtype, [&](auto t) { return dynamics_loops_t<decltype(t)>(w, B, o, dq, dv, dtau, df, dvd, dqd, dlam); });
}
}


static void spec_load(rbd_ws* w, int family, bool force = false);

static bool first_use(rbd_ws* w, SpecKernel& k, bool wanted) {
  if (!wanted || !w->spec_first_use_check || k.checked || capturing(w)) return false;
  k.checked = true;
  return true;
}
struct FirstUseCheck { const char* name; const char* against; const char* quantity; const char* dropped; double floor, tol; };
template <class Reference>
static int first_use_check(rbd_ws* w, const FirstUseCheck& c, long B, const void* out, Layout Lo, size_t tmp_bytes, Reference reference, bool* same) {
  const long n = std::min<long>(B, 256);
  const size_t elems = (size_t)(layout_base(Lo, n - 1) + (long)(w->model->nv - 1) * Lo.sk + 1);
  void *ref = nullptr, *tmp = nullptr;
  double* diff = nullptr;
  HIP_TRY(hipMalloc(&ref, elems * esize(w)));
  if ((tmp_bytes && hipMalloc(&tmp, tmp_bytes) != hipSuccess) || hipMalloc((void**)&diff, 2 * sizeof(double)) != hipSuccess) {
    (void)hipGetLastError(); (void)hipFree(ref); (void)hipFree(tmp); return RBD_ERR_OUT_OF_MEMORY;
// ... 146 lines not shown
    const bool nofext = df == nullptr && w->spec_aba_nofext.f != nullptr;
    SpecKernel* faba = nofext ? &w->spec_aba_nofext : &w->spec_aba;
    const int faba_scratch = nofext ? w->spec_aba_nofext_scratch : w->spec_aba_scratch;
    bool stash_program = false;
    if (spec_f64 && faba->f) {
      SpecKernel* const fg = nofext ? &w->spec_aba_gst_nofext : &w->spec_aba_gst;
      const long waves = (B + 63) / 64, r_lds = (waves + w->spec_ncu - 1) / w->spec_ncu, r_gst = (waves + 2 * w->spec_ncu - 1) / (2 * w->spec_ncu);
      const long ratio = nofext ? w->spec_f64_stash_ratio : w->spec_f64_stash_ratio_fext;
      if (fg->f && (w->spec_f64_stash > 0 || (w->spec_f64_stash < 0 && r_lds * 100 > r_gst * ratio))) { faba = fg; stash_program = true; }
    }
    if (faba->f && (algorithm == RBD_ALGO_ABA_COMPILED || (B >= spec_from && (faba_scratch == 0 || (spec_f64 && faba_scratch <= w->spec_f64_max_scratch))))) {
      Timed t(w);
      long Bl = B;
      const double* gv = gravity ? gravity : m->gravity;
      float gx = (float)gv[0], gy = (float)gv[1], gz = (float)gv[2];
      double gxd = gv[0], gyd = gv[1], gzd = gv[2];
      MkStage F = mk ? *mk : kNoStage;
      void* args[] = {&Bl, &dq, &dv, &dtau, &df, &dvd, &dqd, &Lq, &Lv, &Lf, &gx, &gy, &gz, &F};
      void* stash = nullptr;
      if (w->dtype == RBD_F64) {
        if (stash_program) {
          if (int st = ensure(w->d_rows, sizeof(double) * (size_t)(m->nb + 10 * m->spec_plan().n3) * (size_t)B)) return st;
          stash = w->d_rows.p;
        }
      }
      void* args64[] = {&Bl, &dq, &dv, &dtau, &df, &dvd, &dqd, &Lq, &Lv, &Lf, &gxd, &gyd, &gzd, &F, &stash};
      HIP_TRY(hipModuleLaunchKernel(faba->f, (unsigned)((B + 63) / 64), 1, 1, 64, 1, 1, 0, w->stream, w->dtype == RBD_F64 ? args64 : args, nullptr));
      w->last_kernel = stash_program ? "aba_spec_gst_f64 (compiled for the mechanism at run time; spare rows in the HBM stash)"
                       : w->dtype == RBD_F64 ? "aba_spec_f64 (compiled for the mechanism at run time)" : "aba_spec_f32 (compiled for the mechanism at run time)";
      w->last_aba = stash_program ? ABA_SPEC_STASH : ABA_SPEC;
      bool same = true;
      if (first_use(w, *faba, !mk && dv && dvd))
        if (int st = check_dynamics(w, B, dq, dv, dtau, df, dvd, Lq, Lv, Lf, gravity, &same)) return st;
      if (same) return RBD_OK;
      faba->f = nullptr;
      if (algorithm == RBD_ALGO_ABA_COMPILED) return RBD_ERR_UNSUPPORTED;
    }
  }
  if (algorithm == RBD_ALGO_ABA_COMPILED) return RBD_ERR_UNSUPPORTED;
  int pick = algorithm;
  if (algorithm == RBD_ALGO_ABA) pick = (can_walk && B >= w->walk_min_batch) ? RBD_ALGO_ABA_WALK : (can_bank && B >= w->bank_min_batch) ? RBD_ALGO_ABA_BANKS : RBD_ALGO_ABA_LANES;
  if (algorithm == RBD_ALGO_ABA && pick == RBD_ALGO_ABA_BANKS && can_walk && B >= w->walk_one_round_batch && B >= w->spec_walk_min_batch && (w->dtype == RBD_F64 || w->spec_walk_f32)) {
    const bool no_rr = w->no_reroot;
    if (spec_walk(w, w->walk_rr && !no_rr && w->walk_rr_lds_bytes > 0, 0, 0)) pick = RBD_ALGO_ABA_WALK;
  }
  if (mk && pick != RBD_ALGO_ABA_WALK) return RBD_ERR_UNSUPPORTED;
  Timed t(w);
  w->last_kernel = pick == RBD_ALGO_ABA_BANKS ? "aba_bank_kernel" : "aba_kernel";
  w->last_aba = ABA_OTHER;
  if (pick == RBD_ALGO_ABA_WALK) {
    const bool no_rr = w->no_reroot;
    const int pair = w->dtype == RBD_F32 && w->walk_lds_bytes_pair > 0 && B >= w->walk_pair_min_batch;
    const bool rr = w->walk_rr && !no_rr && (pair ? w->walk_rr_lds_bytes_pair : w->walk_rr_lds_bytes) > 0;
    WalkModel wm = rr ? w->wm_rr : w->wm;
    if (gravity) memcpy(wm.gravity, gravity, sizeof wm.gravity);
    w->last_kernel = pair ? "aba_walk_kernel (two fp32 states per lane)" : "aba_walk_kernel";
    const TrackPlan& TP = rr ? m->rrs.track : m->track;
    const size_t lds = rr ? (pair ? w->walk_rr_lds_bytes_pair : w->walk_rr_lds_bytes) : (pair ? w->walk_lds_bytes_pair : w->walk_lds_bytes);
    const int wkind = (mk && mk->stage == 4) ? 2 : 0;
    if (hipFunction_t f = ((w->dtype == RBD_F64 || w->spec_walk_f32) && (B >= w->spec_walk_min_batch || wkind == 2)) ? spec_walk(w, rr, wkind, pair) : nullptr) {
      w->last_kernel = pair ? "aba_walk_spec (compiled for the mechanism, two fp32 states per lane)" : "aba_walk_spec (compiled for the mechanism)";
      w->last_aba = ABA_WALK_SPEC;
      long Bl = B;
      Layout lq = Lq, lv = Lv, lf = Lf;
      double gx = wm.gravity[0], gy = wm.gravity[1], gz = wm.gravity[2];
      MkStage F = mk ? *mk : kNoStage;
      void* args[] = {&Bl, (void*)&dq, (void*)&dv, (void*)&dtau, (void*)&df, (void*)&dvd, (void*)&dqd, &lq, &lv, &lf, &gx, &gy, &gz, &F};
      const long per = pair ? 128 : 64;
      HIP_TRY(hipModuleLaunchKernel(f, (unsigned)((B + per - 1) / per), 1, 1, 64u * (unsigned)wm.G, 1, 1, 0, w->stream, args, nullptr));
      SpecKernel& k = w->spec_walk[4 * wkind + (rr ? 2 : 0) + (pair ? 1 : 0)];
      bool same = true;
      if (first_use(w, k, !mk && dv && dvd))
        if (int st = check_dynamics(w, B, dq, dv, dtau, df, dvd, Lq, Lv, Lf, gravity, &same)) return st;
      if (!same) { k.f = nullptr; return run_aba(w, B, algorithm, dq, dv, dtau, df, dvd, dqd, Lq, Lv, Lf, gravity, fuse, mk); }
    } else if (mk) {
      return RBD_ERR_UNSUPPORTED;
    } else {
      HIP_TRY(by_dtype(w->dtype, [&](auto t) { return launch_aba_walk<decltype(t)>(wm, TP.has_floating, TP.general, pair, B, lds, dq, dv, dtau, df, dvd, dqd, Lq, Lv, Lf, w->stream); }));
    }
  } else if (pick == RBD_ALGO_ABA_BANKS) {
    BankModel bm = w->bm;
    if (gravity) memcpy(bm.gravity, gravity, sizeof bm.gravity);
    hipFunction_t f = spec_bank(w) ? (fuse ? w->spec_bank_fused : w->spec_bank_aba.f) : nullptr;
    if (f) {
      MkFuse F{};
      F.stage = -1;
      if (fuse) F = *fuse;
      long Bl = B;
      const long spw = 64 / bm.lps, waves = (B + spw - 1) / spw;
      void* args[] = {&bm, &Bl, (void*)&dq, (void*)&dv, (void*)&dtau, (void*)&df, (void*)&dvd, (void*)&dqd, &Lq, &Lv, &Lf, &F};
      HIP_TRY(hipModuleLaunchKernel(f, (unsigned)((waves + 3) / 4), 1, 1, 256, 1, 1, 0, w->stream, args, nullptr));
      w->last_kernel = "aba_bank_kernel (compiled for the mechanism at run time)";
      bool same = true;
      if (first_use(w, w->spec_bank_aba, !fuse && dv && dvd))
        if (int st = check_dynamics(w, B, dq, dv, dtau, df, dvd, Lq, Lv, Lf, gravity, &same)) return st;
      if (!same) { w->spec_bank_aba.f = w->spec_bank_fused = nullptr; return run_aba(w, B, algorithm, dq, dv, dtau, df, dvd, dqd, Lq, Lv, Lf, gravity, fuse, mk); }
    } else {
      HIP_TRY(by_dtype(w->dtype, [&](auto t) { return launch_aba_bank<decltype(t)>(bm, B, dq, dv, dtau, df, dvd, dqd, Lq, Lv, Lf, w->stream, fuse); }));
    }
  } else {
    DevModel dm = w->dm;
    if (gravity) memcpy(dm.gravity, gravity, sizeof dm.gravity);
    HIP_TRY(by_dtype(w->dtype, [&](auto t) { return launch_aba<decltype(t)>(dm, B, dq, dv, dtau, df, dvd, dqd, Lq, Lv, Lf, w->stream, fuse); }));
  }
  return RBD_OK;
}

static bool capturing(rbd_ws* w) {
  hipStreamCaptureStatus cs = hipStreamCaptureStatusNone;
  if (hipStreamIsCapturing(w->stream, &cs) != hipSuccess) { (void)hipGetLastError(); return false; }
  return cs != hipStreamCaptureStatusNone;
}
static void spec_load(rbd_ws* w, int family, bool force) {
  const rbd_model* m = w->model;
  SpecSlot& p = w->spec_prog[spec_slot(family)];
  if (!p.tried && (!m->spec_plan().ok || !spec_has(family, w->dtype, m->nb, m->nq, m->nv, m->spec_plan().n3))) p.tried = true;
  const hipModule_t mod = spec_module(w, p, [&] { return program_source(m, w->dtype, family); }, false, force || !jit_async(), "the interpreting kernels are used");
  if (!mod) return;
  const bool f64 = w->dtype == RBD_F64;
  const int cap = w->spec_max_scratch;
  if (family == SPEC_MASS) {
    w->spec_crba = spec_kernel(mod, f64 ? "crba_spec_f64" : "crba_spec_f32", kNoScratchCheck);
    if (spec_has_chol(w->dtype, m->nv)) {
      w->spec_crba_perm = spec_kernel(mod, "crba_spec_perm_f32", kNoScratchCheck);
      w->spec_chol.f = spec_kernel(mod, "chol_spec_f32", kNoScratchCheck);
      w->spec_chol_packed.f = spec_kernel(mod, "chol_spec_packed_f32", kNoScratchCheck);
      w->spec_chol_nom.f = spec_kernel(mod, "chol_spec_nom_f32", kNoScratchCheck);
      if (!w->spec_chol_nom.f) w->spec_chol.f = nullptr;
      w->spec_emit = spec_kernel(mod, "emit_spec_f32", kNoScratchCheck);
      if (!w->spec_crba_perm || !w->spec_chol.f || !w->spec_emit) w->spec_crba_perm = w->spec_chol.f = w->spec_emit = nullptr;
    } else if (f64 && spec_has_chol(RBD_F32, m->nv)) {
      w->spec_emit = spec_kernel(mod, "emit_spec_f64", kNoScratchCheck);
    }
  } else if (family == SPEC_ABA) {
    const int aba_cap = f64 ? std::max(cap, w->spec_f64_max_scratch) : cap;
    w->spec_aba.f = spec_kernel(mod, f64 ? "aba_spec_f64" : "aba_spec_f32", aba_cap, &w->spec_aba_scratch);
    w->spec_aba_nofext.f = spec_kernel(mod, f64 ? "aba_spec_nofext_f64" : "aba_spec_nofext_f32", aba_cap, &w->spec_aba_nofext_scratch);
    if (f64) {
      w->spec_aba_gst.f = spec_kernel(mod, "aba_spec_gst_f64", aba_cap);
      w->spec_aba_gst_nofext.f = spec_kernel(mod, "aba_spec_gst_nofext_f64", aba_cap);
    }
  } else if (family == SPEC_RNEA) {
    w->spec_rnea.f = spec_kernel(mod, f64 ? "rnea_spec_f64" : "rnea_spec_f32", cap, &w->spec_rnea_scratch);
  } else if (family == SPEC_KIN) {
    w->spec_kin = spec_kernel(mod, f64 ? "kin_spec_f64" : "kin_spec_f32", 0);
    w->spec_jac = spec_kernel(mod, f64 ? "jac_spec_f64" : "jac_spec_f32", 0);
    w->spec_mom = spec_kernel(mod, f64 ? "mom_spec_f64" : "mom_spec_f32", 0);
    w->spec_energy = spec_kernel(mod, f64 ? "energy_spec_f64" : "energy_spec_f32", 0);
    w->spec_com = spec_kernel(mod, f64 ? "com_spec_f64" : "com_spec_f32", 0);
  }
}
static hipError_t launch_kin_spec(rbd_ws* w, hipFunction_t f, long B, const void* q, const void* v, void* A, void* com, void* energy, void* J, unsigned long long jplus,
                                  unsigned long long jminus, void* mom, Layout Lq, Layout Lv, Layout La, Layout L3, Layout L2, Layout L12) {
  void* args[] = {&B, &q, &v, &A, &com, &energy, &J, &jplus, &jminus, &mom, &Lq, &Lv, &La, &L3, &L2, &L12};
  return hipModuleLaunchKernel(f, (unsigned)((B + 63) / 64), 1, 1, 64, 1, 1, 0, w->stream, args, nullptr);
}
static bool spec_crba_fits(const rbd_ws* w) { return (size_t)w->model->nq * 4 * 65 * esize(w) <= 160u * 1024u; }
static hipFunction_t spec_crba(rbd_ws* w, size_t buffer_bytes) {
  spec_load(w, SPEC_MASS);
  return buffer_bytes < ((size_t)1 << 32) && spec_crba_fits(w) ? w->spec_crba : nullptr;
}
static hipError_t launch_crba_spec(rbd_ws* w, hipFunction_t f, long B, const void* q, void* Mout, Layout Lq, Layout Lm, int zero_fill) {
  const unsigned lds = (unsigned)((size_t)w->model->nq * 4 * 65 * esize(w));
  void* args[] = {&B, &q, &Mout, &Lq, &Lm, &zero_fill};
  return hipModuleLaunchKernel(f, (unsigned)((B + 255) / 256), 1, 1, 256, 1, 1, lds, w->stream, args, nullptr);
}

// ... 733 lines not shown
```

### rigidbodydynamics.jl_amd/csrc/rbd_capi_internal.hpp

```cpp
#pragma once
#include <hip/hip_runtime.h>
#include <chrono>
#include <climits>
#include <cmath>
#include <unistd.h>

#include <algorithm>
#include <cstdio>
#include <cstdlib>
#include <cstring>
#include <memory>
#include <new>
#include <string>
#include <vector>

#include "rbd_hip.h"
#include "rbd_internal.hpp"
#include "rbd_chain_plan.hpp"
#include "rbd_track_plan.hpp"
#include "rbd_walk_plan.hpp"
#include "rbd_reroot.hpp"
#include "rbd_state_plan.hpp"
#include "rbd_jit.hpp"
#include "rbd_mk_fuse.hpp"
#include "rbd_tangent.hpp"
#include "rbd_tangent_mk.hpp"
#include "rbd_adjoint.hpp"
#include "rbd_adjoint_mk.hpp"
#include "rbd_point.hpp"
#include "rbd_point_plan.hpp"

using namespace rbd;

#pragma GCC visibility push(hidden)

extern thread_local std::string g_last_hip_error;

#define HIP_TRY(expr)                                                                              \
  do {                                                                                             \
    hipError_t e_ = (expr);                                                                        \
    if (e_ != hipSuccess) {                                                                        \
      g_last_hip_error = std::string(#expr) + ": " + hipGetErrorString(e_);                        \
      return (e_ == hipErrorOutOfMemory) ? RBD_ERR_OUT_OF_MEMORY : RBD_ERR_HIP;                    \
    }                                                                                              \
  } while (0)

template <class F>
auto by_dtype(int dtype, F&& f) { return dtype == RBD_F64 ? f(double()) : f(float()); }

struct rbd_model {
  int32_t nb = 0, nq = 0, nv = 0, nc = 0, nloops = 0;
  int32_t lps = 1, nlevels = 0, maxchild = 0, maxnvj = 0;
  double gravity[3] = {0, 0, 0};
  std::vector<int32_t> ib;
  std::vector<double> rb;
  std::vector<int32_t> nslots;
  uint64_t perm_down = 0;
  int32_t inner_floating = 0, has3dof = 0;
  std::vector<int32_t> slot_of, order;
  std::vector<int32_t> dof_body;
  std::vector<int32_t> anc;
  std::vector<uint64_t> row_mask;
  int32_t row_words = 1;
  std::vector<rbd_loop_joint_t> loops;
  std::vector<int32_t> loop_i, loop_path, jt_ref, voff_ref, parent_ref, qoff_ref;
  std::vector<int32_t> mk1, mkf;
  bool loop_fused_ok = false;
  bool big = false;
  std::vector<int32_t> big_tbl;
  std::vector<double> big_rb;
  std::vector<double> loop_r, axis_ref, axis2_ref;
  int32_t bank_lps = 0, bank_L0 = 0, bank_nb[2] = {0, 0}, bank_aba_ok = 0;
  std::vector<int32_t> bank_ib[2];
  std::vector<double> bank_rb[2];
  uint64_t bank_perm_down = 0;
  ChainPlan chain;
  TrackPlan track;
  Reroot rr;
  struct RrSlots {
    bool ok = false;
    int32_t nlevels = 0;
    std::vector<int32_t> ib, nslots;
    std::vector<double> rb;
    TrackPlan track;
    WalkPlan walk;
  } rrs;
  int32_t ncp = 0, nhs = 0;
  std::vector<int32_t> cp_body;
  std::vector<double> cp_r, hs_r;
  WalkPlan walk;
  StatePlan state;
  StatePlan state_wide;
  const StatePlan& spec_plan() const { return state.ok ? state : state_wide; }
};

struct SpecSlot { bool tried = false; hipModule_t mod = nullptr; std::string src; };
enum { SPEC_LOOP = SPEC_SLOTS, SPEC_BANK, SPEC_WALK, SPEC_PROGRAMS = SPEC_WALK + 12 };
enum AbaProgram { ABA_OTHER, ABA_SPEC, ABA_SPEC_STASH, ABA_WALK_SPEC };
struct SpecKernel { hipFunction_t f = nullptr; bool checked = false; };

struct DevBuf {
  void* p = nullptr;
  size_t bytes = 0;
  DevBuf() = default;
  DevBuf(const DevBuf&) = delete; DevBuf& operator=(const DevBuf&) = delete;
  ~DevBuf() { reset(); }
  void reset() { if (p) (void)hipFree(p); p = nullptr; bytes = 0; }
};

struct rbd_ws {
  const rbd_model* model = nullptr;
  int32_t device = 0, dtype = RBD_F64, max_batch = 0;
  hipStream_t stream = nullptr;
  DevModel dm{};
  BankModel bm{}; DevBuf d_bank_ib[2], d_bank_rb[2];
  DevBuf d_rr_chain_i, d_rr_chain_r;
  WalkModel wm_rr{}; bool walk_rr = false; DevBuf d_rrtrack_ri, d_rrtrack_rr, d_rrwalk_wk; size_t walk_rr_lds_bytes = 0, walk_rr_lds_bytes_pair = 0;
  TrackModel tm{}; DevBuf d_track_ri, d_track_rr;
  ContactModel ctm{}; DevBuf d_cp_body, d_cp_r, d_hs_r;
  DevBuf d_tw, d_s0, d_sacc, d_sdot, d_rows;
  WalkModel wm{}; DevBuf d_walk_wk; size_t walk_lds_bytes = 0, walk_lds_bytes_pair = 0; long walk_min_batch = 0, walk_pair_min_batch = 0, sim_walk_min_batch = 1;
  SpecSlot spec_prog[SPEC_PROGRAMS];
  hipFunction_t spec_kin = nullptr, spec_jac = nullptr, spec_mom = nullptr, spec_energy = nullptr, spec_com = nullptr; long spec_kin_min_batch = (long)1 << 62;
  hipFunction_t spec_crba = nullptr, spec_crba_perm = nullptr, spec_emit = nullptr, spec_loop = nullptr, spec_bank_fused = nullptr;
  SpecKernel spec_chol, spec_chol_nom, spec_chol_packed;
  SpecKernel spec_aba, spec_aba_nofext, spec_aba_gst, spec_aba_gst_nofext, spec_rnea;
  SpecKernel spec_bank_aba, spec_bank_rnea;
  SpecKernel spec_walk[12];
  int spec_f64_max_scratch = 0;
  int spec_f64_stash = -1, spec_f64_stash_ratio = 170, spec_f64_stash_ratio_fext = 120, spec_ncu = 256;
  bool spec_first_use_check = true, spec_first_use_inject = false;
  int spec_aba_scratch = 0, spec_aba_nofext_scratch = 0, spec_rnea_scratch = 0;
  bool no_reroot = false, loop_no_fused = false; int spec_max_scratch = 512;
  bool spec_walk_f32 = true;
  std::vector<double> loop_gains; bool custom_gains = false;
  void* bound_M = nullptr; void* bound_c = nullptr;
  long spec_aba_min_batch = 0, spec_rnea_min_batch = 0, spec_walk_min_batch = 0, walk_one_round_batch = 0, rnea_walk_min_batch = 0;
  StateModel sm{}; DevBuf d_state_ops, d_state_cols, d_state_sr; long state_min_batch = 0; long mass_min_batch = (long)1 << 62, mass_solve_min_batch = (long)1 << 62; long spec_aba_fused_min_batch = (long)1 << 62; long sim_walk_max_batch = 0; bool state_aot = false;
  DevBuf d_Msoa; long Msoa_B = -1; int Msoa_perm = -1;
  long bank_min_batch = 0, rnea_bank_min_batch = 0, bank_resident_states = 0;
  DevBuf d_ib, d_rb, d_dof_body, d_anc, d_row_mask;
  DevBuf stage[8];
  DevBuf d_M, d_c, d_K, d_k;
  DevBuf d_body, d_scratch;
  BigModel big{}; DevBuf d_big_tbl, d_big_rb, d_big_scratch, d_big_L;
  DevBuf d_fused_i;
  DevBuf d_loop_i, d_loop_r, d_loop_path, d_jt_ref, d_voff_ref, d_axis_ref, d_axis2_ref;
  MkBuffers mk{}; DevBuf d_mk_q0, d_mk_v0, d_mk_phid[4], d_mk_vd[4], d_vdwork; size_t mk_elems = 0;
  DevBuf d_tauwork;
  DevBuf d_notpd;
  int32_t result_layout = RBD_LAYOUT_SOA; int32_t result_B = 0;
  int32_t timing = 0;
  hipEvent_t ev0 = nullptr, ev1 = nullptr;
  bool ev_pending = false;
  const char* last_kernel = "";
  int last_aba = ABA_OTHER;
  bool tan_ready = false; BigModel tan{}; DevBuf d_tan_tbl, d_tan_rb, d_tan_scratch; long tan_threads = 0; int tan_ntan = 0;
  DevBuf d_tan_M, d_tan_L, d_tan_c, d_tan_vd, d_tan_rhs, d_tan_x;
  DevBuf d_sim_val, d_sim_tan; int sim_tan_w = 0;
  bool adj_ready = false; long adj_states = 0;
  DevBuf d_adj_scratch, d_adj_rhs, d_adj_lam, d_adj_x;
  bool sav_ready = false; int sav_nn = 0, sav_nw = 0;
  DevBuf d_sav_joints, d_sav, d_sav_ckpt;
  bool tan_tbl_ready = false; PointPlan pts{}; DevBuf d_pt_i, d_pt_r;
  bool ct_ready = false; PointPlan ct_pts{}; DevBuf d_ct_i, d_ct_r, d_ct_pbar, d_ct_vbar, d_ct_wbar, d_ct_s;
  bool sct_ready = false; DevBuf d_sct;
  ~rbd_ws() {
    (void)hipSetDevice(device);
    for (const SpecSlot& p : spec_prog) if (p.mod) (void)hipModuleUnload(p.mod);
    if (ev0) (void)hipEventDestroy(ev0);
    if (ev1) (void)hipEventDestroy(ev1);
  }
};

long tune(const char* key, long dflt, bool* has = nullptr);

inline size_t esize(const rbd_ws* w) { return w->dtype == RBD_F64 ? 8 : 4; }

inline Layout layout_of(int layout, long n, long B) {
  Layout L;
  if (layout == RBD_LAYOUT_AOS) { L.sk = 1; L.sb = n; } else { L.sk = B; L.sb = 1; }
  return L;
}

inline bool missing(const void* p, long n) { return p == nullptr && n > 0; }

struct Opts { int layout, memory, algorithm, stabilization; };

const bool kAnySize = true, kUpTo64Bodies = false;
inline int begin_call(rbd_ws* w, int32_t B, const rbd_opts_t* opts, bool any_size, Opts* o) {
  *o = opts ? Opts{opts->layout, opts->memory, opts->algorithm, opts->stabilization} : Opts{RBD_LAYOUT_SOA, RBD_MEM_DEVICE, RBD_ALGO_ABA, 1};
  if (!w) return RBD_ERR_INVALID_ARGUMENT;
  if (w->model->big && !any_size) return RBD_ERR_UNSUPPORTED;
  if (B < 0 || B > w->max_batch) return RBD_ERR_DIMENSION_MISMATCH;
  if (o->layout != RBD_LAYOUT_SOA && o->layout != RBD_LAYOUT_AOS) return RBD_ERR_INVALID_ARGUMENT;
  if (o->memory != RBD_MEM_DEVICE && o->memory != RBD_MEM_HOST) return RBD_ERR_INVALID_ARGUMENT;
  return RBD_OK;
}

struct Timed {
  rbd_ws* w;
  explicit Timed(rbd_ws* w_) : w(w_) { if (w->timing) (void)hipEventRecord(w->ev0, w->stream); }
  ~Timed() { if (w->timing) { (void)hipEventRecord(w->ev1, w->stream); w->ev_pending = true; } }
};

int ensure(DevBuf& b, size_t need);
int upload(DevBuf& dst, const void* src, size_t bytes);
int upload_real(DevBuf& dst, const std::vector<double>& src, int dtype);

class HostIO {
// ... 41 lines not shown
```

### rigidbodydynamics.jl_amd/csrc/rbd_jit.hip

```cpp
#include <dlfcn.h>
#include <hip/hip_runtime.h>
#include <hip/hiprtc.h>
#include <sys/stat.h>
#include <unistd.h>

#include <cstdio>
#include <cstdlib>
#include <algorithm>
#include <cstring>
#include <atomic>
#include <map>
#include <memory>
#include <mutex>
#include <thread>
#include <string>
#include <vector>

#include "rbd_internal.hpp"
#include "rbd_jit.hpp"
#include "rbd_walk_plan.hpp"
#include "rbd_jit_embed.inc"

namespace rbd {

// ... 436 lines not shown
    snprintf(b, sizeof b, "  __shared__ __align__(16) %s rnea_lds[%d];\n  rbd::spec::rnea_spec<%s, %s>(B, q, v, vdot, fext, tau, Lq, Lv, Lf, acc_out, jw_out, Lo, rnea_lds);\n}\n", T,
             (dtype == RBD_F32 ? nq + 2 * nv : nq) * 65, T, dtype == RBD_F32 ? "false" : "true");
    s += b;
  }
  if (aba) {
    for (int gst = 0; gst <= (dtype == RBD_F64 ? 1 : 0); ++gst) {
      const int udl = dtype == RBD_F64 ? aba_udl(nb, nq, nv, P.n3, gst) : 0;
      char lds[160];
      snprintf(lds, sizeof lds, "  __shared__ __align__(16) %s aba_lds[%d];\n", T,
               (dtype == RBD_F64 ? aba_f64_rows(nb, nq, nv, P.n3, gst) + udl * nb : nq + 2 * nv + std::max(nq, nb) + 10 * P.n3) * 65);
      for (int fx = 1; fx >= 0; --fx) {
        snprintf(b, sizeof b, "extern \"C\" __global__ __launch_bounds__(64) void aba_spec_%s%s%s(long B, const %s* q, const %s* v, const %s* tau, const %s* fext, %s* vdot,\n"
                 "                                                            %s* qdot, rbd::Layout Lq, rbd::Layout Lv, rbd::Layout Lf, %s gx, %s gy, %s gz, rbd::MkStage F%s) {\n",
                 gst ? "gst_" : "", fx ? "" : "nofext_", sfx, T, T, T, T, T, T, T, T, T, dtype == RBD_F64 ? ", double* stash" : "");
        s += b;
        s += lds;
        snprintf(b, sizeof b, "  rbd::spec::aba_spec<%s, %s, %d, %d>(B, q, v, tau, %s, vdot, qdot, Lq, Lv, Lf, gx, gy, gz, aba_lds, F%s);\n}\n", T, fx ? "true" : "false", udl, gst,
                 fx ? "fext" : "nullptr", dtype == RBD_F64 ? ", stash" : "");
        s += b;
      }
    }
  }
  if (chol) {
    s += "extern \"C\" __global__ __launch_bounds__(256) void crba_spec_perm_f32(long B, const float* q, float* M, rbd::Layout Lq, rbd::Layout Lm, int zero_fill) {\n"
         "  extern __shared__ __align__(16) unsigned char spec_lds[];\n"
         "  rbd::spec::crba_spec<float, true>(B, q, M, Lq, Lm, zero_fill, reinterpret_cast<float*>(spec_lds));\n}\n";
    s += "extern \"C\" __global__ __launch_bounds__(64, RBD_SPEC_CHOL_WAVES) void chol_spec_f32(long B, const float* Mg, const float* tau, const float* c, float* x, rbd::Layout Lv,\n"
         "                                                                   int* notpd, float* Mcopy, rbd::Layout Lc) {\n"
         "  __shared__ __align__(16) float mst[rbd::spec::chol_emit_lds()];\n"
         "  rbd::spec::chol_spec<false, true>(B, blockIdx.x, Mg, tau, c, x, Lv, notpd, Mcopy, Lc, mst);\n}\n";
    s += "extern \"C\" __global__ __launch_bounds__(64, RBD_SPEC_CHOL_WAVES) void chol_spec_nom_f32(long B, const float* Mg, const float* tau, const float* c, float* x, rbd::Layout Lv,\n"
         "                                                                       int* notpd, float* Mcopy, rbd::Layout Lc) {\n"
         "  rbd::spec::chol_spec<false, false>(B, blockIdx.x, Mg, tau, c, x, Lv, notpd, nullptr, Lc, nullptr);\n}\n";
    s += "extern \"C\" __global__ __launch_bounds__(64, RBD_SPEC_CHOL_WAVES) void chol_spec_packed_f32(long B, const float* Mg, const float* tau, const float* c, float* x, rbd::Layout Lv,\n"
         "                                                                          int* notpd, float* Mcopy, rbd::Layout Lc) {\n"
         "  __shared__ __align__(16) float mst[rbd::spec::chol_emit_lds()];\n"
         "  rbd::spec::chol_spec<true, true>(B, blockIdx.x, Mg, tau, c, x, Lv, notpd, Mcopy, Lc, mst);\n}\n";
  }
  if (emit) {
    snprintf(b, sizeof b, "extern \"C\" __global__ __launch_bounds__(64, 2) void emit_spec_%s(long B, const %s* Mg, %s* Mcopy, rbd::Layout Lc) {\n"
                          "  __shared__ __align__(16) %s mst[16 * rbd::spec::emit_mst<%s>()];\n  rbd::spec::emit_spec<%s>(B, blockIdx.x, Mg, Mcopy, Lc, mst);\n}\n", sfx, T, T, T, T, T);
    s += b;
  }
  return s;
}

std::string spec_loop_source(const LoopTables& L, int dtype) {
  if (!(L.nloops > 0 && L.nb <= 4 && L.nv <= 4 && L.nc <= 6 && L.nv < L.nc)) return std::string();
  const char* T = dtype == RBD_F32 ? "float" : "double";
  const char* sfx = dtype == RBD_F32 ? "f32" : "f64";
  std::string s;
  char b[1024];
  s += "// generated by rbd_jit.hip: the loop tables of one small mechanism as constants (rbd_loop_small.hpp)\n#include \"rbd_loop_small.hpp\"\nnamespace rbd_loop_plan {\n";
  auto ints = [&](const char* name, const std::vector<int32_t>& v) {
    snprintf(b, sizeof b, "__device__ const int32_t %s[%d] = ", name, (int)std::max<size_t>(v.size(), 1));
    s += b;
    if (v.empty()) s += "{0}"; else put_ints(s, v.data(), (int)v.size());
    s += ";\n";
  };
  auto reals = [&](const char* name, const std::vector<double>& v) {
    snprintf(b, sizeof b, "__device__ const %s %s[%d] = ", T, name, (int)std::max<size_t>(v.size(), 1));
    s += b;
    if (v.empty()) s += "{0}"; else put_reals(s, v.data(), (int)v.size());
    s += ";\n";
  };
  ints("LI", *L.li); ints("PATH", *L.path); ints("JT", *L.jt); ints("VOFF", *L.voff); ints("XI", *L.xi);
  reals("LR", *L.lr); reals("AXIS", *L.axis); reals("AXIS2", *L.axis2); reals("RB", *L.rb);
  snprintf(b, sizeof b, "struct View {\n  static constexpr int nloops = %d, nc = %d, nv = %d, nb = %d;\n", L.nloops, L.nc, L.nv, L.nb);
  s += b;
  snprintf(b, sizeof b, "  const int32_t* li = LI; const %s* lr = LR; const int32_t* path = PATH; const int32_t* jt = JT; const int32_t* voff = VOFF;\n"
                        "  const %s* axis = AXIS; const %s* axis2 = AXIS2; const int32_t* xi = XI; const %s* rb = RB; const %s* gains = nullptr;\n};\n}  // namespace rbd_loop_plan\n", T, T, T, T, T);
  s += b;
  snprintf(b, sizeof b, "extern \"C\" __global__ __launch_bounds__(64) void loop_spec_%s(long B, int stabilize, const %s* q, const %s* v, const %s* tau, const %s* fext,\n"
                        "    %s* Mg, %s* cg, %s* vdot, %s* qdot, %s* lambda, %s* Kg, %s* kg, rbd::Layout Lq, rbd::Layout Lm, rbd::Layout Lv, rbd::Layout Lf, rbd::Layout Lc,\n"
                        "    rbd::Layout Lk, int* notpd, const %s* gains) {\n", sfx, T, T, T, T, T, T, T, T, T, T, T, T);
  s += b;
  s += "  const long st = (long)blockIdx.x * blockDim.x + threadIdx.x;\n  if (st >= B) return;\n  rbd_loop_plan::View V;\n  V.gains = gains;  // nullptr: the model's gains, compile-time constants\n";
  snprintf(b, sizeof b, "  rbd::loop_fused_small_state<%s, rbd_loop_plan::View, %d, %d, %d, true>(V, st, stabilize, q, v, tau, fext, Mg, Mg, cg, vdot, qdot, lambda, Kg, kg,\n"
                        "      Lq, Lm, Lv, Lf, Lc, Lk, %.17g, %.17g, %.17g, notpd);\n}\n", T, L.nb, L.nv, L.nc, L.gravity[0], L.gravity[1], L.gravity[2]);
  s += b;
  return s;
}

std::string spec_bank_source(int nlevels, int L0, const int32_t* nslots, unsigned long long perm_down, int simple, int dtype) {
  if (nlevels < 2 || nlevels > 64 || L0 < 1 || L0 >= nlevels) return std::string();
  const char* T = dtype == RBD_F32 ? "float" : "double";
  const char* sfx = dtype == RBD_F32 ? "f32" : "f64";
  const char* SI = simple ? "true" : "false";
  std::string s;
  char b[1600];
  s += "// generated by rbd_jit.hip: the level structure of one mechanism for the banked kernels (aba_bank_body / rnea_bank_body, rbd_bank.hpp): loops over the levels unrolled,\n"
       "// DPP hop or exchange column and the number of later children known per level\n";
  snprintf(b, sizeof b, "#define RBD_BANK_FIXED_NL %d\n#define RBD_BANK_FIXED_L0 %d\n#define RBD_BANK_FIXED_PERM 0x%llxull\n#define RBD_BANK_FIXED_NS ", nlevels, L0, perm_down);
  s += b;
  for (int l = 0; l < nlevels; ++l) { snprintf(b, sizeof b, "%s%d", l ? "," : "", (int)nslots[l]); s += b; }
  s += "\n#include \"rbd_lane.hpp\"\n#include \"rbd_bank.hpp\"\n";
  const char* lds = "  __shared__ __align__(16) unsigned char lds[(size_t)rbd::BANK_LDS_PAIRS * 256 * sizeof(rbd::Pair2<%s>)];\n";
  for (int fused = 0; fused < 2; ++fused) {
    snprintf(b, sizeof b, "extern \"C\" __global__ __launch_bounds__(256, RBD_BANK_WAVES) void aba_bank_%sspec_%s(rbd::BankModel M, long B, const %s* q, const %s* v, const %s* tau,\n"
                          "    const %s* fext, %s* vdot, %s* qdot, rbd::Layout Lq, rbd::Layout Lv, rbd::Layout Lf, rbd::MkFuse F) {\n",
             fused ? "fused_" : "", sfx, T, T, T, T, T, T);
    s += b;
    snprintf(b, sizeof b, lds, T);
    s += b;
    snprintf(b, sizeof b, "  rbd::aba_bank_body<%s, %s, %s>(M, B, q, v, tau, fext, vdot, qdot, Lq, Lv, Lf, F, reinterpret_cast<rbd::Pair2<%s>*>(lds));\n}\n", T, fused ? "true" : "false", SI, T);
    s += b;
  }
  snprintf(b, sizeof b, "extern \"C\" __global__ __launch_bounds__(256, 2) void rnea_bank_spec_%s(rbd::BankModel M, long B, int ncol, const %s* q, const %s* v, const %s* vdot, const %s* fext,\n"
                        "    %s* tau, %s* qdot, rbd::Layout Lq, rbd::Layout Lv, rbd::Layout Lf, %s* acc_out, %s* jw_out) {\n"
                        "  __shared__ __align__(16) unsigned char lds[(size_t)rbd::RNEA_LDS_PAIRS * 256 * sizeof(rbd::Pair2<%s>)];\n"
                        "  rbd::rnea_bank_body<%s, %s>(M, B, ncol, q, v, vdot, fext, tau, qdot, Lq, Lv, Lf, acc_out, jw_out, reinterpret_cast<rbd::Pair2<%s>*>(lds));\n}\n",
           sfx, T, T, T, T, T, T, T, T, T, T, SI, T);
  s += b;
  return s;
}

size_t walk_spec_lds_bytes(const WalkTables& W, int dtype, int pair) {
  return walk_rows(W.nq, W.nv, W.nA, W.nB, W.nS) * WR_STRIDE * ((dtype == RBD_F64 || pair) ? 8 : 4);
}
bool walk_spec_has(int dtype, int ns, int G, size_t lds_rows_bytes) {
  return (dtype == RBD_F64 || dtype == RBD_F32) && ns >= 1 && ns <= WALK_MAX_STEPS && G >= 1 && G <= 4 && lds_rows_bytes <= 160 * 1024;
}
const char* walk_spec_suffix(int dtype, int pair) { return dtype == RBD_F64 ? "f64" : pair ? "f32x2" : "f32"; }
std::string walk_spec_source(const WalkTables& W, int dtype, int kind, int pair) {
  if (dtype == RBD_F64) pair = 0;
  const size_t lds = walk_spec_lds_bytes(W, dtype, pair);
  if (!walk_spec_has(dtype, W.ns, W.G, lds)) return std::string();
  const char* S = dtype == RBD_F64 ? "double" : "float";
  const char* T = dtype == RBD_F64 ? "double" : pair ? "rbd::f2" : "float";
  const char* sfx = walk_spec_suffix(dtype, pair);
  std::string s;
  char b[1400];
  {
    const char* e = getenv("RBD_TUNE"); const char* k = e ? strstr(e, "spec_variant=") : nullptr;
    if (k && (atol(k + 13) & 32)) s += "#define RBD_WALK_ABLATE_OUT_LOCAL 1\n";
    if (k && (atol(k + 13) & 256)) s += "#define RBD_WALK_NO_STAGE 1\n";
  }
  if (kind == 2) {
    snprintf(b, sizeof b, "// rbd-walk-sim-loop stash-from=a%d\n// rbd-jit-option: -mllvm\n// rbd-jit-option: -disable-machine-licm\n",
             256 - ((dtype == RBD_F64 || pair) ? 2 : 1) * W.ns * WALK_STASH_N);
    s += b;
  }
  s += "// generated by rbd_jit.hip: the walk plan of one mechanism as constants (aba_walk_spec / rnea_walk_spec, rbd_walk.hpp)\n#include \"rbd_walk.hpp\"\nnamespace rbd_walk_tables {\n";
  const int nrec = W.ns * W.G;
  snprintf(b, sizeof b, "__device__ const int32_t RI[%d] __attribute__((aligned(16))) = ", nrec * TI_STRIDE);
  s += b; put_ints(s, W.ri->data(), nrec * TI_STRIDE); s += ";\n";
  snprintf(b, sizeof b, "__device__ const %s RR[%d] = ", S, nrec * TR_STRIDE);
  s += b; put_reals(s, W.rrc->data(), nrec * TR_STRIDE); s += ";\n";
  snprintf(b, sizeof b, "__device__ const int32_t WK[%d] = ", nrec);
  s += b; put_ints(s, W.wk->data(), nrec); s += ";\n";
  const int nch = W.rr ? W.nchain : 0;
  snprintf(b, sizeof b, "__device__ const int32_t CHI[%d] = ", std::max(nch, 1) * 4);
  s += b; if (nch) put_ints(s, W.chain_i->data(), nch * 4); else s += "{0, 0, 0, 0}"; s += ";\n";
  snprintf(b, sizeof b, "__device__ const %s CHR[%d] = ", S, std::max(nch, 1) * 15);
  s += b; if (nch) put_reals(s, W.chain_r->data(), nch * 15); else s += "{0}"; s += ";\n";
  const int n1 = W.mk1 ? (int)W.mk1->size() / 3 : 0, nf = W.mkf ? (int)W.mkf->size() / 2 : 0;
  snprintf(b, sizeof b, "__device__ const int32_t MK1[%d] = ", std::max(3 * n1, 1));
  s += b; if (n1) put_ints(s, W.mk1->data(), 3 * n1); else s += "{0}"; s += ";\n";
  snprintf(b, sizeof b, "__device__ const int32_t MKF[%d] = ", std::max(2 * nf, 1));
  s += b; if (nf) put_ints(s, W.mkf->data(), 2 * nf); else s += "{0}"; s += ";\n";
  int fw = 0, fewest = 1 << 30;
  for (int g = 0; g < W.G; ++g) {
    int n = 0;
    for (int st = 0; st < W.ns; ++st) n += ((*W.ri)[((size_t)st * W.G + g) * TI_STRIDE + TI_W1] >> 16) & TF_VALID ? 1 : 0;
    if (n < fewest) { fewest = n; fw = g; }
  }
  snprintf(b, sizeof b, "struct Plan {\n  static constexpr int NS = %d, G = %d, NQ = %d, NV = %d, MK_N1 = %d, MK_NF = %d, MK_FW = %d;\n  static constexpr unsigned long long SFM_AW = 0x%llxull, SFM_BW = 0x%llxull;\n",
           W.ns, W.G, W.nq, W.nv, n1, nf, fw, (unsigned long long)W.sfm[1], (unsigned long long)W.sfm[3]);
  s += b;
  s += "  static __device__ __forceinline__ rbd::WalkModel model() {\n    rbd::WalkModel M{};\n";
  snprintf(b, sizeof b, "    M.ns = %d; M.G = %d; M.nA = %d; M.nB = %d; M.nS = %d; M.nq = %d; M.nv = %d;\n    M.ri = RI; M.rr = RR; M.wk = WK;\n", W.ns, W.G, W.nA, W.nB, W.nS,
           W.nq, W.nv);
  s += b;
  for (int k = 0; k < 5; ++k) { snprintf(b, sizeof b, "    M.sfm[%d] = 0x%llxull;\n", k, (unsigned long long)W.sfm[k]); s += b; }
  if (nch) {
    snprintf(b, sizeof b, "    M.reroot.nchain = %d; M.reroot.fq = %d; M.reroot.fv = %d; M.reroot.chain_i = CHI; M.reroot.chain_r = CHR;\n", nch, W.fq, W.fv);
    s += b;
    for (int k = 0; k < 12; ++k) { snprintf(b, sizeof b, "    M.reroot.fXp[%d] = %.17g;\n", k, W.fXp[k]); s += b; }
  }
  s += "    return M;\n  }\n};\n}  // namespace rbd_walk_tables\n";
  if (kind == 0 || kind == 2)
    snprintf(b, sizeof b, "extern \"C\" __global__ __launch_bounds__(%d) void aba_walk_%sspec_%s(long B, const %s* q, const %s* v, const %s* tau, const %s* fext,\n"
                          "    %s* vdot, %s* qdot, rbd::Layout Lq, rbd::Layout Lv, rbd::Layout Lf, double gx, double gy, double gz, rbd::MkStage F) {\n"
                          "  __shared__ __align__(16) unsigned char lds[%zu];\n"
                          "  rbd::aba_walk_spec<%s, %s, %s, %s, rbd_walk_tables::Plan, %s>(B, q, v, tau, fext, vdot, qdot, Lq, Lv, Lf, gx, gy, gz, lds, F, rbd_walk_tables::MK1, rbd_walk_tables::MKF);\n}\n",
             64 * W.G, kind == 2 ? "sim_" : "", sfx, S, S, S, S, S, S, lds, T, W.flt ? "true" : "false", W.gen ? "true" : "false", nch ? "true" : "false", kind == 2 ? "true" : "false");
  else
    snprintf(b, sizeof b, "extern \"C\" __global__ __launch_bounds__(%d) void rnea_walk_spec_%s(long B, const %s* q, const %s* v, const %s* vdot, const %s* fext,\n"
                          "    %s* tau, %s* qdot, rbd::Layout Lq, rbd::Layout Lv, rbd::Layout Lf, %s* acc_out, %s* jw_out, double gx, double gy, double gz) {\n"
                          "  __shared__ __align__(16) unsigned char lds[%zu];\n"
                          "  rbd::rnea_walk_spec<%s, %s, %s, rbd_walk_tables::Plan>(B, q, v, vdot, fext, tau, qdot, Lq, Lv, Lf, acc_out, jw_out, gx, gy, gz, lds);\n}\n",
             64 * W.G, sfx, S, S, S, S, S, S, S, S, lds, T, W.flt ? "true" : "false", W.gen ? "true" : "false");
  s += b;
  return s;
}

// ... 290 lines not shown
```

### rigidbodydynamics.jl_amd/csrc/rbd_jit.hpp

```cpp
#pragma once
#include <cstdint>
#include <string>
#include <vector>

#include "rbd_state_plan.hpp"

namespace rbd {
bool jit_available();
enum { SPEC_MASS = 0, SPEC_ABA = 1, SPEC_RNEA = 2, SPEC_FAMILIES = 3 };
enum { SPEC_KIN = 11, SPEC_SLOTS = 4 };
inline int spec_slot(int family) { return family == SPEC_KIN ? 3 : family; }
bool spec_has(int family, int dtype, int nb, int nq, int nv, int n3 = 0);
bool spec_has_chol(int dtype, int nv);
std::string spec_source(const StatePlan& P, int nb, int nq, int nv, const uint64_t* row_mask, const double* gravity, int dtype, int family);
struct LoopTables {
  int nb, nq, nv, nc, nloops;
  const std::vector<int32_t>*li, *path, *jt, *voff, *xi;
  const std::vector<double>*lr, *axis, *axis2, *rb;
  const double* gravity;
};
std::string spec_loop_source(const LoopTables& L, int dtype);
std::string spec_bank_source(int nlevels, int L0, const int32_t* nslots, unsigned long long perm_down, int simple, int dtype);
struct WalkTables {
  int ns, G, nA, nB, nS, nq, nv, flt, gen, rr;
  const std::vector<int32_t>*ri, *wk;
  const std::vector<double>* rrc;
  uint64_t sfm[5];
  int nchain, fq, fv;
  const std::vector<int32_t>* chain_i;
  const std::vector<double>* chain_r;
  const double* fXp;
  const std::vector<int32_t>*mk1, *mkf;
};
bool walk_spec_has(int dtype, int ns, int G, size_t lds_rows_bytes);
size_t walk_spec_lds_bytes(const WalkTables& W, int dtype, int pair = 0);
const char* walk_spec_suffix(int dtype, int pair);
std::string walk_spec_source(const WalkTables& W, int dtype, int kind = 0, int pair = 0);
enum { JIT_READY = 0, JIT_PENDING = 1, JIT_FAILED = 2 };
bool jit_async();
void jit_wait_idle();
int jit_code_object_get(const std::string& source, bool wait, std::vector<char>* code, std::string* log);
int jit_walk_code_object_get(const std::string& source, bool wait, std::vector<char>* code, std::string* log);
int jit_kd_cover_agprs(std::vector<char>* code);
bool jit_walk_admit(const std::string& source, std::vector<char>* code, std::string* log);
std::vector<char> jit_walk_code_object(const std::string& source, std::string* log);
std::vector<char> jit_code_object(const std::string& source, std::string* log);
void jit_cache_discard(const std::string& source);
}
```

### rigidbodydynamics.jl_amd/state.py

```python
from __future__ import annotations

import ctypes
from typing import Optional

import numpy as np
import torch

from . import _capi
from .mechanism import FlatModel, Mechanism, flatten


class DimensionMismatch(ValueError):
    """Julia's DimensionMismatch (e.g. src/mechanism_algorithms.jl:250)."""


def _raise(status, where):
    try:
        _capi.check(status, where)
    except _capi.RBDError as e:
        if e.status == 2:
            raise DimensionMismatch(str(e)) from None
        if e.status == 1:
            raise ValueError(str(e)) from None
        if e.status == 7:
# ... 740 lines not shown
        for _ in range(nsteps):
            _raise(L.rbd_simulate(state.ws.handle, state.batch, _ptr(state.q), _ptr(state.v), _ptr(torques), _ptr(externalwrenches),
                                  ctypes.c_double(dt), 1, ctypes.byref(opts)), "rbd_simulate")
            qs.append(state.q.clone())
            vs.append(state.v.clone())
    else:
        tau = torch.zeros_like(state.v) if torques is None else torques
        vd = torch.zeros_like(state.v)
        lam = torch.zeros((state.batch, max(f.nc, 1)), dtype=state.dtype, device=state.device)
        for k in range(nsteps):
            for stage in range(5):
                _raise(L.rbd_mk_stage(state.ws.handle, state.batch, stage, ctypes.c_double(dt), _ptr(state.q), _ptr(state.v),
                                      _ptr(vd if stage > 0 else None), ctypes.byref(opts)), "rbd_mk_stage")
                if stage < 4:
                    control_(tau, ts[k] + RK4_C[stage] * dt, state)
                    _raise(L.rbd_dynamics(state.ws.handle, state.batch, _ptr(state.q), _ptr(state.v), _ptr(tau), _ptr(externalwrenches),
                                          _ptr(vd), None, _ptr(lam if f.nc else None), ctypes.byref(opts)), "rbd_dynamics")
            if store:
                qs.append(state.q.clone())
                vs.append(state.v.clone())
    ts = np.array(ts)
    return (ts, qs, vs) if store else ts


def dynamics_ode_(xd: torch.Tensor, result: DynamicsResult, state: MechanismState, x: torch.Tensor, torques: Optional[torch.Tensor] = None,
                  externalwrenches: Optional[torch.Tensor] = None, stabilization_gains="default"):
    f = state.flat
    ns = getattr(f, "ns", 0)
    if state.layout != "aos":
        raise ValueError("dynamics_ode_ expects the AOS layout (one state vector per row)")
    n = f.nq + f.nv + ns
    if tuple(x.shape) != (state.batch, n) or tuple(xd.shape) != (state.batch, n):
        raise DimensionMismatch(f"x / ẋ must be ({state.batch}, {n}) = [q; v{'; s' if ns else ''}]")
    state.q.copy_(x[:, :f.nq])
    state.v.copy_(x[:, f.nq:f.nq + f.nv])
    if ns:
        state.s.copy_(x[:, f.nq + f.nv:])
    dynamics_(result, state, torques, externalwrenches, stabilization_gains=stabilization_gains)
    xd[:, :f.nq].copy_(result.qd)
    xd[:, f.nq:f.nq + f.nv].copy_(result.vd)
    if ns:
        xd[:, f.nq + f.nv:].copy_(result.sd)
    return xd


def _kin(state: MechanismState, A=None, com=None, energy=None):
    state.ws.use_current_stream()
    opts = state._opts()
    _raise(_capi.lib().rbd_kinematics(state.ws.handle, state.batch, _ptr(state.q), _ptr(state.v), _ptr(A), _ptr(com), _ptr(energy),
                                      ctypes.byref(opts)), "rbd_kinematics")


def momentum_matrix_(out: torch.Tensor, state: MechanismState):
    state._check(out, 6 * state.flat.nv, "momentum matrix")
    _kin(state, A=out)
    return out


def center_of_mass(state: MechanismState) -> torch.Tensor:
    out = state._zeros(3)
    _kin(state, com=out)
    return out


def kinetic_energy(state: MechanismState) -> torch.Tensor:
    e = state._zeros(2)
    _kin(state, energy=e)
    return e[:, 0] if state.layout == "aos" else e[0]


def gravitational_potential_energy(state: MechanismState) -> torch.Tensor:
    e = state._zeros(2)
    _kin(state, energy=e)
    return e[:, 1] if state.layout == "aos" else e[1]


def jit_source(flat, dtype=torch.float32, family="mass_matrix"):
    L = _capi.lib()
    h = ctypes.c_void_p()
    _raise(L.rbd_model_create(ctypes.cast(ctypes.byref(flat.c_struct()), ctypes.c_void_p), ctypes.byref(h)), "rbd_model_create")
    try:
        dt = _capi.F64 if dtype == torch.float64 else _capi.F32
        fam = {"mass_matrix": 0, "dynamics": 1, "inverse_dynamics": 2, "loops": 3, "dynamics_tracks": 4, "inverse_dynamics_tracks": 5, "dynamics_tracks_pairs": 6,
               "inverse_dynamics_tracks_pairs": 7, "banked": 8, "dynamics_tracks_sim": 9, "dynamics_tracks_pairs_sim": 10, "kinematics": 11}[family]
        n = L.rbd_jit_source(h, dt, fam, None, 0)
        if n < 0:
            return None
        buf = ctypes.create_string_buffer(n + 1)
        L.rbd_jit_source(h, dt, fam, buf, n + 1)
        return buf.value.decode()
    finally:
        L.rbd_model_destroy(h)


def jit_precompile(flat, dtype=torch.float32):
    L = _capi.lib()
    h = ctypes.c_void_p()
    _raise(L.rbd_model_create(ctypes.cast(ctypes.byref(flat.c_struct()), ctypes.c_void_p), ctypes.byref(h)), "rbd_model_create")
    try:
        log = ctypes.create_string_buffer(1 << 16)
        st = L.rbd_jit_precompile(h, _capi.F64 if dtype == torch.float64 else _capi.F32, log, len(log))
        return (None if st == 3 else st == 0), log.value.decode(errors="replace")
    finally:
        L.rbd_model_destroy(h)


def jit_status(flat, dtype=torch.float32, family: int = 0) -> int:
    L = _capi.lib()
    h = ctypes.c_void_p()
    _raise(L.rbd_model_create(ctypes.cast(ctypes.byref(flat.c_struct()), ctypes.c_void_p), ctypes.byref(h)), "rbd_model_create")
    try:
        return int(L.rbd_jit_status(h, _capi.F64 if dtype == torch.float64 else _capi.F32, int(family)))
    finally:
        L.rbd_model_destroy(h)


def chain_plan(flat):
    import numpy as np
    L = _capi.lib()
    h = ctypes.c_void_p()
    _raise(L.rbd_model_create(ctypes.cast(ctypes.byref(flat.c_struct()), ctypes.c_void_p), ctypes.byref(h)), "rbd_model_create")
    try:
        g, ns, nf = ctypes.c_int32(), ctypes.c_int32(), ctypes.c_int32()
        st = L.rbd_model_chain_plan(h, ctypes.byref(g), ctypes.byref(ns), ctypes.byref(nf), None, 0)
        if st == 3:
            return None
        _raise(st, "rbd_model_chain_plan")
        tab = np.zeros(ns.value * g.value, np.int32)
        _raise(L.rbd_model_chain_plan(h, None, None, None, tab.ctypes.data_as(ctypes.POINTER(ctypes.c_int32)), tab.size), "rbd_model_chain_plan")
        return {"tracks": g.value, "steps": ns.value, "lds_fields": nf.value, "table": tab.reshape(ns.value, g.value)}
    finally:
        L.rbd_model_destroy(h)


def reroot_plan(flat):
    import numpy as np
    L = _capi.lib()
    h = ctypes.c_void_p()
    _raise(L.rbd_model_create(ctypes.cast(ctypes.byref(flat.c_struct()), ctypes.c_void_p), ctypes.byref(h)), "rbd_model_create")
    try:
        dims = np.zeros(12, np.int32)
        pi = lambda a: a.ctypes.data_as(ctypes.POINTER(ctypes.c_int32))
        pd = lambda a: a.ctypes.data_as(ctypes.POINTER(ctypes.c_double))
        st = L.rbd_model_reroot_plan(h, pi(dims), None, 0, None, 0, None, 0, None, None, None)
        if st == 3:
            return None
        _raise(st, "rbd_model_reroot_plan")
        n, nch = int(dims[0]) * int(dims[1]), int(dims[7])
        ri, rr, wk = np.zeros(n * 4 + int(dims[1]), np.int32), np.zeros(n * 24, np.float64), np.zeros(n, np.int32)
        ci, cr, fxp = np.zeros(max(4 * nch, 1), np.int32), np.zeros(max(15 * nch, 1), np.float64), np.zeros(12, np.float64)
        _raise(L.rbd_model_reroot_plan(h, None, pi(ri), ri.size, pd(rr), rr.size, pi(wk), wk.size, pi(ci), pd(cr), pd(fxp)), "rbd_model_reroot_plan")
        return {"tracks": int(dims[0]), "steps": int(dims[1]), "root": int(dims[10]), "floating_body": int(dims[11]), "chain": nch, "dims": dims,
                "ri": ri, "rr": rr, "wk": wk, "chain_i": ci, "chain_r": cr, "fxp": fxp}
    finally:
        L.rbd_model_destroy(h)


def track_plan(flat):
    import numpy as np
    L = _capi.lib()
    h = ctypes.c_void_p()
    _raise(L.rbd_model_create(ctypes.cast(ctypes.byref(flat.c_struct()), ctypes.c_void_p), ctypes.byref(h)), "rbd_model_create")
    try:
        dims = np.zeros(6, np.int32)
        pi = lambda a: a.ctypes.data_as(ctypes.POINTER(ctypes.c_int32))
        st = L.rbd_model_track_plan(h, pi(dims), None, 0, None, 0, None, 0)
        if st == 3:
# ... 143 lines not shown
```

Measured before the change: 217.3 million.

## Run banked ABA on the mechanism re-rooted at its centre

```diff
diff --git a/rigidbodydynamics.jl_amd/csrc/rbd_bank.hpp b/rigidbodydynamics.jl_amd/csrc/rbd_bank.hpp
--- a/rigidbodydynamics.jl_amd/csrc/rbd_bank.hpp
+++ b/rigidbodydynamics.jl_amd/csrc/rbd_bank.hpp
@@ -30,6 +30,28 @@
 #endif
 
 namespace rbd {
+#ifdef RBD_BANK_RR
+__device__ const int32_t kBankRrChainI[] = {RBD_BANK_RR_CHAIN_I};
+__device__ const double kBankRrChainR[] = {RBD_BANK_RR_CHAIN_R};
+constexpr bool kBankRr = true;
+constexpr int kBankRrFbBank = RBD_BANK_RR_FB_BANK;
+RBD_DEV RerootView bank_rr_view() {
+  RerootView V{};
+  const double f[12] = {RBD_BANK_RR_FXP};
+  V.nchain = RBD_BANK_RR_NCHAIN; V.fq = RBD_BANK_RR_FQ; V.fv = RBD_BANK_RR_FV;
+  V.chain_i = kBankRrChainI; V.chain_r = kBankRrChainR;
+#pragma unroll
+  for (int k = 0; k < 12; ++k) V.fXp[k] = f[k];
+  return V;
+}
+#else
+constexpr bool kBankRr = false;
+constexpr int kBankRrFbBank = 0;
+RBD_DEV RerootView bank_rr_view() { return RerootView{}; }
+#endif
+}
+
+namespace rbd {
 
 template <typename T> struct alignas(2 * sizeof(T)) Pair2 { T a, b; };
 
@@ -56,7 +78,7 @@
   for (int k = 0; k < N; k += 6) massign6(mask, d + k, s + k);
 }
 
-enum { PK_KIN = 0, PK_FWD = 6, PARK_PAIRS = 16, PK_XCH = 16, XCH_PAIRS = 14, BANK_LDS_PAIRS = PARK_PAIRS + XCH_PAIRS };
+enum { PK_KIN = 0, PK_FWD = 6, PK_RRF = 13, PARK_PAIRS = 16, PK_XCH = 16, XCH_PAIRS = 14, BANK_LDS_PAIRS = PARK_PAIRS + XCH_PAIRS };
 
 template <typename T, int N> RBD_DEV void lds_put(Pair2<T>* col, int pair0, const T* x) {
 #pragma unroll
@@ -278,9 +300,11 @@
                            const T* __restrict__ fext, T* __restrict__ vdot, T* __restrict__ qdot, Layout Lq, Layout Lv, Layout Lf, const MkFuse& F,
                            Pair2<T>* const lds) {
   Pair2<T>* const col = lds + threadIdx.x;
+  constexpr bool RR = kBankRr && !FUSED;
+  static_assert(!RR || SIMPLE, "the re-rooted form is written for revolute tree joints");
   RBD_MARK(0);
   BankRegs<T> r0, r1;
-  auto fetch = [&](int k, BankRegs<T>& c, T* qj, T* vj) {
+  auto fetch = [&](int k, BankRegs<T>& c, T* qj, T* vj, T* cq, T* cv ) {
     load_bank_body(M, k, B, c.b);
     c.rb = reinterpret_cast<const T*>(M.rb[k]) + (c.b.sub < M.nbk[k] ? c.b.sub : 0) * RB_STRIDE;
     c.pcol = (int)threadIdx.x - c.b.sub + (c.b.parent >= 0 ? c.b.parent : c.b.sub);
@@ -310,13 +334,28 @@
           for (int k2 = 1; k2 < 6; ++k2) c.tj[k2] = tau[va + k2 * Lv.sk];
         }
       }
+      if (RR && k == 0) {
+#pragma unroll
+        for (int j = 0; j < RC_MAX; ++j) { cq[j] = T(0); cv[j] = T(0); }
+        if (fl) {
+          RBD_KEEP_BRANCH();
+          const RerootView V = bank_rr_view();
+#pragma unroll
+          for (int j = 0; j < RC_MAX; ++j)
+            if (j < V.nchain) {
+              cq[j] = q[(long)V.chain_i[4 * j + 1] * Lq.sk + sc * Lq.sb];
+              if (hv) cv[j] = v[(long)V.chain_i[4 * j + 2] * Lv.sk + sc * Lv.sb];
+            }
+        }
+      }
     } else {
       load_joint_q(c.b, q, Lq, qj);
       load_joint_v(c.b, v, Lv, vj);
       load_joint_v(c.b, tau, Lv, c.tj);
     }
   };
-  auto setup = [&](BankRegs<T>& c, T* qj, T* vj, T* XR, T* Xp, T* tl, T* ta ) {
+  auto setup = [&](BankRegs<T>& c, T* qj, T* vj, T* XR, T* Xp, T* tl, T* ta , const T* cq, const T* cv) {
+    T rtw[6] = {T(0), T(0), T(0), T(0), T(0), T(0)};
     if (SIMPLE) {
       const bool fl = c.b.jtype == RBD_JOINT_QUAT_FLOATING;
       const T ax[3] = {c.rb[RB_AXIS], c.rb[RB_AXIS + 1], c.rb[RB_AXIS + 2]};
@@ -344,6 +383,14 @@
 #pragma unroll
           for (int k = 0; k < 7; ++k) qdot[(long)(c.b.qoff + k) * Lq.sk + c.b.state * Lq.sb] = o[k];
         }
+        if (RR && cq != nullptr) {
+          const RerootView V = bank_rr_view();
+          T Rf[9], pf[3], wf[6];
+          reroot_fb_pose(V, qj, Rf, pf);
+          xforce(Rf, pf, c.tj, wf);
+          lds_put<T, 6>(col, PK_RRF, wf);
+          reroot_root_kinematics<T, double>(V, qj, vj, cq, cv, Rj, pj, rtw);
+        }
       } else if (qdot != nullptr && c.b.valid) {
         qdot[(long)c.b.qoff * Lq.sk + c.b.state * Lq.sb] = vj[0];
       }
@@ -366,6 +413,13 @@
 #pragma unroll
     for (int i = 0; i < 3; ++i) c.p()[i] = Xp[i];
     xmotion(c.R(), c.p(), tl, c.Tw());
+    if (RR) {
+      if (c.b.jtype == RBD_JOINT_QUAT_FLOATING) {
+        RBD_KEEP_BRANCH();
+#pragma unroll
+        for (int i = 0; i < 6; ++i) c.Tw()[i] = rtw[i];
+      }
+    }
     if (SIMPLE) {
       c.K[18] = ta[3];
       c.K[19] = T(0);
@@ -415,12 +469,50 @@
     for (int i = 0; i < 6; ++i) c.U[i] = T(0);
     c.Dinv = T(0);
     c.u = T(0);
-    if (floating) xforce(c.R(), c.p(), c.tj, c.U);
+    if (floating && !RR) xforce(c.R(), c.p(), c.tj, c.U);
   };
+  auto rr_take_joint_force = [&](BankRegs<T>& c) {
+    if (RR) {
+      if (c.b.valid && (c.b.flags & BFD_FCARRY)) {
+        RBD_KEEP_BRANCH();
+        T wf[6];
+        lds_get<T, 6>(lds + ((int)threadIdx.x - c.b.sub), PK_RRF, wf);
+#pragma unroll
+        for (int i = 0; i < 6; ++i) c.pA[i] -= wf[i];
+      }
+    }
+  };
+  auto rr_floating_vdot = [&](BankRegs<T>& c, bool bank1) {
+    if (RR) {
+      if (c.b.valid && (c.b.flags & BFD_FCARRY)) {
+        RBD_KEEP_BRANCH();
+        const RerootView V = bank_rr_view();
+        T Rf[9], pf[3], d[6], vf[6];
+        if (!bank1) {
+          T k12[12];
+          lds_get<T, 12>(col, PK_KIN, k12);
+          reroot_fb_pose_from_rebased<T, double>(V, k12, k12 + 9, Rf, pf);
+        } else {
+          T q7[7];
+#pragma unroll
+          for (int k = 0; k < 7; ++k) q7[k] = q[(long)(V.fq + k) * Lq.sk + c.b.state * Lq.sb];
+          reroot_fb_pose(V, q7, Rf, pf);
+        }
+#pragma unroll
+        for (int k = 0; k < 3; ++k) { d[k] = c.acc[k]; d[3 + k] = c.acc[3 + k] + T(M.gravity[k]); }
+        xmotion_inv(Rf, pf, d, vf);
+        if (vdot) {
+#pragma unroll
+          for (int k = 0; k < 6; ++k) vdot[(long)(V.fv + k) * Lv.sk + c.b.state * Lv.sb] = vf[k];
+        }
+      }
+    }
+  };
 
   T qj0[7], vj0[6], qj1[7], vj1[6];
-  fetch(0, r0, qj0, vj0);
-  fetch(1, r1, qj1, vj1);
+  T cq0[RC_MAX], cv0[RC_MAX];
+  fetch(0, r0, qj0, vj0, cq0, cv0);
+  fetch(1, r1, qj1, vj1, nullptr, nullptr);
   if (FUSED) {
     if (F.close_prev) {
       mk_stage_lane(r0.b, 4, (T)F.dt, qj0, vj0, (const T*)nullptr, F.W, (T*)F.q_state, (T*)F.v_state, Lq, Lv);
@@ -433,7 +525,7 @@
   }
   {
     T XR[9], Xp[3], tl[6], ta[4];
-    setup(r0, qj0, vj0, XR, Xp, tl, ta);
+    setup(r0, qj0, vj0, XR, Xp, tl, ta, cq0, cv0);
     RBD_MARK(1);
 RBD_BANK_UNROLL
     for (int l = 1; l < RBD_BK_L0; ++l) bank_fk_step<T, SIMPLE>(M, l, RBD_BK_PERM(l), r0, lds, XR, Xp, SIMPLE ? ta : tl);
@@ -441,7 +533,7 @@
   {
     T XR[9], Xp[3], tl[6], ta[4];
     RBD_MARK(2);
-    setup(r1, qj1, vj1, XR, Xp, tl, ta);
+    setup(r1, qj1, vj1, XR, Xp, tl, ta, nullptr, nullptr);
     RBD_MARK(3);
     lds_put<T, (SIMPLE ? 20 : 24)>(col, PK_KIN, r0.K);
     wave_lds_sync();
@@ -451,6 +543,7 @@
   }
   RBD_MARK(4);
   terms(r1, false);
+  if (kBankRrFbBank == 1) rr_take_joint_force(r1);
   RBD_MARK(5);
 
   NsStream nss = ns_begin(M.ns_desc);
@@ -466,6 +559,7 @@
   for (int i = 0; i < 21; ++i) r0.IA[i] = T(0);
 #pragma unroll
   for (int i = 0; i < 6; ++i) r0.pA[i] = T(0);
+  if (kBankRrFbBank == 0) rr_take_joint_force(r0);
   bank_handoff<T, 1>(RBD_BK_L0, RBD_BK_NS(RBD_BK_L0), r1, r0, lds);
   {
     lds_get<T, (SIMPLE ? 20 : 24)>(col, PK_KIN, r0.K);
@@ -498,12 +592,14 @@
       RBD_KEEP_BRANCH();
       T rhs[6], d[6], k12[12];
 #pragma unroll
-      for (int i = 0; i < 6; ++i) rhs[i] = c.U[i] - c.pA[i];
+      for (int i = 0; i < 6; ++i) rhs[i] = RR ? -c.pA[i] : c.U[i] - c.pA[i];
       sym6_solve(c.IA, rhs, fa);
-#pragma unroll
-      for (int i = 0; i < 6; ++i) d[i] = fa[i] - a0[i];
-      lds_get<T, 12>(col, PK_KIN, k12);
-      xmotion_inv(k12, k12 + 9, d, fv);
+      if (!RR) {
+#pragma unroll
+        for (int i = 0; i < 6; ++i) d[i] = fa[i] - a0[i];
+        lds_get<T, 12>(col, PK_KIN, k12);
+        xmotion_inv(k12, k12 + 9, d, fv);
+      }
     }
     massign<T, 6>(fl0, c.acc, fa);
     massign<T, 6>(fl0, c.vd, fv);
@@ -512,6 +608,10 @@
 RBD_BANK_UNROLL
   for (int l = 1; l < RBD_BK_L0; ++l) bank_accel_step<T>(M, l, RBD_BK_PERM(l), r0, lds);
   RBD_MARK(10);
+  if (RR) {
+    if (r0.b.flags & BFD_VROOT) r0.b.valid = false;
+    if (kBankRrFbBank == 0) rr_floating_vdot(r0, false);
+  }
   if (vdot) store_joint_v(r0.b, vdot, Lv, r0.vd);
   if (FUSED) store_joint_v(r0.b, (T*)F.W.vd[F.stage], Lv, r0.vd);
   {
@@ -539,6 +639,7 @@
 RBD_BANK_UNROLL
   for (int l = RBD_BK_L0 + 1; l < RBD_BK_NL; ++l) bank_accel_step<T>(M, l, RBD_BK_PERM(l), r1, lds);
   RBD_MARK(11);
+  if (RR && kBankRrFbBank == 1) rr_floating_vdot(r1, true);
   if (vdot) store_joint_v(r1.b, vdot, Lv, r1.vd);
   if (FUSED) store_joint_v(r1.b, (T*)F.W.vd[F.stage], Lv, r1.vd);
 }
diff --git a/rigidbodydynamics.jl_amd/csrc/rbd_capi.hip b/rigidbodydynamics.jl_amd/csrc/rbd_capi.hip
--- a/rigidbodydynamics.jl_amd/csrc/rbd_capi.hip
+++ b/rigidbodydynamics.jl_amd/csrc/rbd_capi.hip
@@ -1,4 +1,5 @@
 #include "rbd_capi_internal.hpp"
+static const long kBankRerootDefault[2] = {1, 1};
 enum { BANK_LDS_PAIRS_HOST = 30 };
 
 thread_local std::string g_last_hip_error;
@@ -40,9 +41,44 @@
   return dflt;
 }
 
+static BankSplit bank_split(int nb, int nlevels, const std::vector<int32_t>& ib, const std::vector<double>& rb) {
+  BankSplit S;
+  auto level = [&](int s) { return ib[(size_t)s * IB_STRIDE + IB_LEVEL]; };
+  std::vector<int> per_level(nlevels, 0);
+  for (int s = 0; s < nb; ++s) per_level[level(s)]++;
+  int best_L0 = 0, best_lanes = 1 << 30, best_diff = 1 << 30;
+  for (int L0 = 1; L0 < nlevels; ++L0) {
+    int cA = 0, cB = 0;
+    for (int l = 0; l < nlevels; ++l) (l < L0 ? cA : cB) += per_level[l];
+    int lanes = 1;
+    while (lanes < std::max(cA, cB)) lanes <<= 1;
+    const int diff = std::abs(cA - cB);
+    if (lanes < best_lanes || (lanes == best_lanes && diff < best_diff)) { best_lanes = lanes; best_L0 = L0; best_diff = diff; }
+  }
+  S.lps = best_lanes; S.L0 = best_L0;
+  std::vector<int> bslot(nb, -1);
+  int cnt[2] = {0, 0};
+  for (int s = 0; s < nb; ++s) bslot[s] = cnt[level(s) >= best_L0]++;
+  S.nb[0] = cnt[0]; S.nb[1] = cnt[1];
+  for (int k = 0; k < 2; ++k) { S.ib[k].assign((size_t)std::max(cnt[k], 1) * IB_STRIDE, -1); S.rb[k].assign((size_t)std::max(cnt[k], 1) * RB_STRIDE, 0.0); }
+  for (int s = 0; s < nb; ++s) {
+    const int k = level(s) >= best_L0, j = bslot[s];
+    const int32_t* src = &ib[(size_t)s * IB_STRIDE];
+    int32_t* dst = &S.ib[k][(size_t)j * IB_STRIDE];
+    memcpy(dst, src, sizeof(int32_t) * IB_STRIDE);
+    const int ps = src[IB_PARENT];
+    dst[IB_PARENT] = ps < 0 ? -1 : bslot[ps];
+    for (int c2 = 0; c2 < src[IB_NCHILD]; ++c2) dst[IB_CHILD0 + c2] = bslot[src[IB_CHILD0 + c2]];
+    if (ps >= 0 && level(s) != best_L0 && bslot[ps] != j - 1) { S.perm_down |= (uint64_t)1 << level(s); dst[IB_FLAGS] |= BFD_NOTFIRST; }
+    memcpy(&S.rb[k][(size_t)j * RB_STRIDE], &rb[(size_t)s * RB_STRIDE], sizeof(double) * RB_STRIDE);
+  }
+  return S;
+}
+
 static std::string loop_program_source(const rbd_model* m, int dtype, std::vector<int32_t>* xi_store);
 static int bank_simple(const rbd_model* m);
 static std::string bank_program_source(const rbd_model* m, int dtype, int simple);
+static std::string bank_rr_program_source(const rbd_model* m, int dtype);
 static std::string walk_program_source(const rbd_model* m, int dtype, bool rerooted, int kind = 0, int pair = 0);
 static bool walk_program_rerooted(const rbd_model* m, int dtype, int pair = 0);
 
@@ -50,7 +86,8 @@
 
 int rbd_version(void) { return RBD_HIP_H_VERSION; }
 static std::string program_source(const rbd_model* m, int32_t dtype, int32_t family) {
-  if (!m || (dtype != RBD_F32 && dtype != RBD_F64) || family < 0 || family > SPEC_KIN) return std::string();
+  if (!m || (dtype != RBD_F32 && dtype != RBD_F64) || family < 0 || family > SPEC_BANK_RR_FAMILY) return std::string();
+  if (family == SPEC_BANK_RR_FAMILY) return bank_rr_program_source(m, dtype);
   if (family == SPEC_KIN) return m->spec_plan().ok ? spec_source(m->spec_plan(), m->nb, m->nq, m->nv, m->row_mask.data(), m->gravity, dtype, SPEC_KIN) : std::string();
   if (family == SPEC_FAMILIES + 6) return walk_program_source(m, dtype, walk_program_rerooted(m, dtype), 2);
   if (family == SPEC_FAMILIES + 7) return dtype == RBD_F32 ? walk_program_source(m, dtype, walk_program_rerooted(m, dtype, 1), 2, 1) : std::string();
@@ -98,7 +135,7 @@
   if ((!m->spec_plan().ok && !m->loop_fused_ok && !(m->track.ok && m->walk.ok) && m->bank_lps <= 0) || !jit_available()) return RBD_ERR_UNSUPPORTED;
   struct Job { std::string src; bool walk; int family; int state; double seconds; std::string log; };
   std::vector<Job> jobs;
-  for (int family : {4, 9, 5, 6, 10, 7, 8, 0, 1, 2, 11, 3})
+  for (int family : {4, 9, 5, 6, 10, 7, 8, 12, 0, 1, 2, 11, 3})
     jobs.push_back({program_source(m, dtype, family), family_is_walk(family), family, JIT_PENDING, 0.0, std::string()});
   int part = 0, parts = 1;
   if (const char* e = getenv("RBD_JIT_PRECOMPILE_PART")) { if (sscanf(e, "%d/%d", &part, &parts) != 2 || parts < 1 || part < 0 || part >= parts) { part = 0; parts = 1; } }
@@ -381,36 +418,10 @@
   if (int lst = build_loop_tables(m, d)) { delete m; return lst; }
   m->bank_aba_ok = (m->nloops == 0 && !m->has3dof && !m->inner_floating);
   if (m->nlevels >= 2) {
-    std::vector<int> per_level(m->nlevels, 0);
-    for (int s = 0; s < nb; ++s) per_level[level[s]]++;
-    int best_L0 = 0, best_lanes = 1 << 30, best_diff = 1 << 30;
-    for (int L0 = 1; L0 < m->nlevels; ++L0) {
-      int cA = 0, cB = 0;
-      for (int l = 0; l < m->nlevels; ++l) (l < L0 ? cA : cB) += per_level[l];
-      int lanes = 1;
-      while (lanes < std::max(cA, cB)) lanes <<= 1;
-      const int diff = std::abs(cA - cB);
-      if (lanes < best_lanes || (lanes == best_lanes && diff < best_diff)) { best_lanes = lanes; best_L0 = L0; best_diff = diff; }
-    }
-    if (best_lanes < m->lps) {
-      m->bank_lps = best_lanes; m->bank_L0 = best_L0;
-      std::vector<int> bslot(nb, -1);
-      int cnt[2] = {0, 0};
-      for (int s = 0; s < nb; ++s) bslot[s] = cnt[level[s] >= best_L0]++;
-      m->bank_nb[0] = cnt[0]; m->bank_nb[1] = cnt[1];
-      for (int k = 0; k < 2; ++k) { m->bank_ib[k].assign((size_t)std::max(cnt[k], 1) * IB_STRIDE, -1); m->bank_rb[k].assign((size_t)std::max(cnt[k], 1) * RB_STRIDE, 0.0); }
-      m->bank_perm_down = 0;
-      for (int s = 0; s < nb; ++s) {
-        const int k = level[s] >= best_L0, j = bslot[s];
-        const int32_t* src = &m->ib[(size_t)s * IB_STRIDE];
-        int32_t* dst = &m->bank_ib[k][(size_t)j * IB_STRIDE];
-        memcpy(dst, src, sizeof(int32_t) * IB_STRIDE);
-        const int ps = src[IB_PARENT];
-        dst[IB_PARENT] = ps < 0 ? -1 : bslot[ps];
-        for (int c2 = 0; c2 < src[IB_NCHILD]; ++c2) dst[IB_CHILD0 + c2] = bslot[src[IB_CHILD0 + c2]];
-        if (ps >= 0 && level[s] != best_L0 && bslot[ps] != j - 1) { m->bank_perm_down |= (uint64_t)1 << level[s]; dst[IB_FLAGS] |= BFD_NOTFIRST; }
-        memcpy(&m->bank_rb[k][(size_t)j * RB_STRIDE], &m->rb[(size_t)s * RB_STRIDE], sizeof(double) * RB_STRIDE);
-      }
+    BankSplit bs = bank_split(nb, m->nlevels, m->ib, m->rb);
+    if (bs.lps < m->lps) {
+      m->bank_lps = bs.lps; m->bank_L0 = bs.L0; m->bank_perm_down = bs.perm_down;
+      for (int k = 0; k < 2; ++k) { m->bank_nb[k] = bs.nb[k]; m->bank_ib[k].swap(bs.ib[k]); m->bank_rb[k].swap(bs.rb[k]); }
     }
   }
   {
@@ -485,6 +496,8 @@
               if (e >= 0) S.walk.wk[k] |= S.ib[(size_t)e * IB_STRIDE + IB_FLAGS] << 8;
             }
         }
+        if (S.nlevels >= 2) S.bank = bank_split(nb, S.nlevels, S.ib, S.rb);
+        S.bank_ok = m->bank_lps > 0 && S.bank.lps > 0 && S.bank.lps <= m->bank_lps && R.depth_after < R.depth_before && S.nlevels == R.depth_after && bank_simple(m);
         S.ok = true;
       }
     }
@@ -694,6 +707,18 @@
     V.nchain = (int32_t)(R.chain_i.size() / RC_I_STRIDE); V.fq = R.fq; V.fv = R.fv;
     V.chain_i = (const int32_t*)w->d_rr_chain_i.p; V.chain_r = w->d_rr_chain_r.p;
     memcpy(V.fXp, R.fXp, sizeof V.fXp);
+    if (st == RBD_OK && S.bank_ok && w->bm.simple) {
+      BankModel& br = w->bm_rr;
+      br = w->bm;
+      for (int k = 0; k < 2 && st == RBD_OK; ++k) {
+        st = upload(w->d_bank_rr_ib[k], S.bank.ib[k].data(), S.bank.ib[k].size() * sizeof(int32_t));
+        if (st == RBD_OK) st = upload_real(w->d_bank_rr_rb[k], S.bank.rb[k], dtype);
+        br.ib[k] = (const int32_t*)w->d_bank_rr_ib[k].p; br.rb[k] = w->d_bank_rr_rb[k].p; br.nbk[k] = S.bank.nb[k];
+      }
+      br.lps = S.bank.lps; br.nlevels = S.nlevels; br.L0 = S.bank.L0; br.perm_down = S.bank.perm_down;
+      nslots_pack_desc(br.ns_desc, S.nslots.data(), S.nlevels);
+      w->bank_rr = st == RBD_OK && tune("bank_no_reroot", 0) == 0 && tune("bank_reroot", kBankRerootDefault[dtype == RBD_F64 ? 1 : 0]) != 0;
+    }
     if (st == RBD_OK && S.track.ok && S.walk.ok) {
       const TrackPlan& P = S.track;
       st = upload(w->d_rrtrack_ri, P.ri.data(), P.ri.size() * sizeof(int32_t));
@@ -939,6 +964,19 @@
   if (m->bank_lps <= 0) return std::string();
   return spec_bank_source(m->nlevels, m->bank_L0, m->nslots.data(), (unsigned long long)m->bank_perm_down, simple, dtype);
 }
+static std::string bank_rr_program_source(const rbd_model* m, int dtype) {
+  if (!m->rrs.ok || !m->rrs.bank_ok || tune("bank_generic", 0)) return std::string();
+  const Reroot& R = m->rr;
+  const BankSplit& K = m->rrs.bank;
+  int fb_bank = -1;
+  for (int k = 0; k < 2; ++k)
+    for (int j = 0; j < K.nb[k]; ++j)
+      if (K.ib[k][(size_t)j * IB_STRIDE + IB_FLAGS] & BFD_FCARRY) fb_bank = k;
+  if (fb_bank < 0) return std::string();
+  const BankRrTables T{m->rrs.nlevels, K.L0, (int)(R.chain_i.size() / RC_I_STRIDE), R.fq, R.fv, fb_bank, m->rrs.nslots.data(), (unsigned long long)K.perm_down,
+                       R.chain_i.data(), R.chain_r.data(), R.fXp};
+  return spec_bank_rr_source(T, dtype);
+}
 static std::string loop_program_source(const rbd_model* m, int dtype, std::vector<int32_t>* xi_store) {
   if (!m->loop_fused_ok) return std::string();
   xi_store->assign(3 * (size_t)m->nb, 0);
@@ -1026,6 +1064,15 @@
     w->spec_bank_rnea.f = spec_kernel(mod, ("rnea_bank_spec_" + sfx).c_str(), w->spec_max_scratch);
   }
   return w->spec_bank_aba.f != nullptr;
+}
+
+static hipFunction_t spec_bank_rr(rbd_ws* w) {
+  SpecSlot& p = w->spec_prog[SPEC_BANK_RR];
+  if (!w->bank_rr) p.tried = true;
+  if (hipModule_t mod = spec_module(w, p, [&] { return bank_rr_program_source(w->model, w->dtype); }, false, !jit_async(),
+                                    "the banked kernels of the original tree are used"))
+    w->spec_bank_rr.f = spec_kernel(mod, w->dtype == RBD_F64 ? "aba_bank_rr_spec_f64" : "aba_bank_rr_spec_f32", w->spec_max_scratch);
+  return w->spec_bank_rr.f;
 }
 
 namespace {
@@ -1338,7 +1385,22 @@
     BankModel bm = w->bm;
     if (gravity) memcpy(bm.gravity, gravity, sizeof bm.gravity);
     hipFunction_t f = spec_bank(w) ? (fuse ? w->spec_bank_fused : w->spec_bank_aba.f) : nullptr;
-    if (f) {
+    hipFunction_t frr = (f && !fuse && !mk && w->bank_rr) ? spec_bank_rr(w) : nullptr;
+    if (frr) {
+      BankModel br = w->bm_rr;
+      memcpy(br.gravity, bm.gravity, sizeof br.gravity);
+      MkFuse F{};
+      F.stage = -1;
+      long Bl = B;
+      const long spw = 64 / br.lps, waves = (B + spw - 1) / spw;
+      void* args[] = {&br, &Bl, (void*)&dq, (void*)&dv, (void*)&dtau, (void*)&df, (void*)&dvd, (void*)&dqd, &Lq, &Lv, &Lf, &F};
+      HIP_TRY(hipModuleLaunchKernel(frr, (unsigned)((waves + 3) / 4), 1, 1, 256, 1, 1, 0, w->stream, args, nullptr));
+      w->last_kernel = "aba_bank_kernel (compiled for the mechanism at run time, tree re-rooted at its centre)";
+      bool same = true;
+      if (first_use(w, w->spec_bank_rr, dv && dvd))
+        if (int st = check_dynamics(w, B, dq, dv, dtau, df, dvd, Lq, Lv, Lf, gravity, &same)) return st;
+      if (!same) { w->spec_bank_rr.f = nullptr; w->bank_rr = false; return run_aba(w, B, algorithm, dq, dv, dtau, df, dvd, dqd, Lq, Lv, Lf, gravity, fuse, mk); }
+    } else if (f) {
       MkFuse F{};
       F.stage = -1;
       if (fuse) F = *fuse;
diff --git a/rigidbodydynamics.jl_amd/csrc/rbd_capi_internal.hpp b/rigidbodydynamics.jl_amd/csrc/rbd_capi_internal.hpp
--- a/rigidbodydynamics.jl_amd/csrc/rbd_capi_internal.hpp
+++ b/rigidbodydynamics.jl_amd/csrc/rbd_capi_internal.hpp
@@ -47,6 +47,13 @@
 
 template <class F>
 auto by_dtype(int dtype, F&& f) { return dtype == RBD_F64 ? f(double()) : f(float()); }
+
+struct BankSplit {
+  int32_t lps = 0, L0 = 0, nb[2] = {0, 0};
+  std::vector<int32_t> ib[2];
+  std::vector<double> rb[2];
+  uint64_t perm_down = 0;
+};
 
 struct rbd_model {
   int32_t nb = 0, nq = 0, nv = 0, nc = 0, nloops = 0;
@@ -84,6 +91,8 @@
     std::vector<double> rb;
     TrackPlan track;
     WalkPlan walk;
+    BankSplit bank;
+    bool bank_ok = false;
   } rrs;
   int32_t ncp = 0, nhs = 0;
   std::vector<int32_t> cp_body;
@@ -95,7 +104,7 @@
 };
 
 struct SpecSlot { bool tried = false; hipModule_t mod = nullptr; std::string src; };
-enum { SPEC_LOOP = SPEC_SLOTS, SPEC_BANK, SPEC_WALK, SPEC_PROGRAMS = SPEC_WALK + 12 };
+enum { SPEC_LOOP = SPEC_SLOTS, SPEC_BANK, SPEC_WALK, SPEC_BANK_RR = SPEC_WALK + 12 , SPEC_PROGRAMS };
 enum AbaProgram { ABA_OTHER, ABA_SPEC, ABA_SPEC_STASH, ABA_WALK_SPEC };
 struct SpecKernel { hipFunction_t f = nullptr; bool checked = false; };
 
@@ -114,6 +123,7 @@
   hipStream_t stream = nullptr;
   DevModel dm{};
   BankModel bm{}; DevBuf d_bank_ib[2], d_bank_rb[2];
+  BankModel bm_rr{}; DevBuf d_bank_rr_ib[2], d_bank_rr_rb[2]; bool bank_rr = false;
   DevBuf d_rr_chain_i, d_rr_chain_r;
   WalkModel wm_rr{}; bool walk_rr = false; DevBuf d_rrtrack_ri, d_rrtrack_rr, d_rrwalk_wk; size_t walk_rr_lds_bytes = 0, walk_rr_lds_bytes_pair = 0;
   TrackModel tm{}; DevBuf d_track_ri, d_track_rr;
@@ -126,6 +136,7 @@
   SpecKernel spec_chol, spec_chol_nom, spec_chol_packed;
   SpecKernel spec_aba, spec_aba_nofext, spec_aba_gst, spec_aba_gst_nofext, spec_rnea;
   SpecKernel spec_bank_aba, spec_bank_rnea;
+  SpecKernel spec_bank_rr;
   SpecKernel spec_walk[12];
   int spec_f64_max_scratch = 0;
   int spec_f64_stash = -1, spec_f64_stash_ratio = 170, spec_f64_stash_ratio_fext = 120, spec_ncu = 256;
diff --git a/rigidbodydynamics.jl_amd/csrc/rbd_jit.hip b/rigidbodydynamics.jl_amd/csrc/rbd_jit.hip
--- a/rigidbodydynamics.jl_amd/csrc/rbd_jit.hip
+++ b/rigidbodydynamics.jl_amd/csrc/rbd_jit.hip
@@ -542,6 +542,25 @@
   return s;
 }
 
+namespace {
+void bank_level_defines(std::string& s, int nlevels, int L0, const int32_t* nslots, unsigned long long perm_down) {
+  char b[400];
+  snprintf(b, sizeof b, "#define RBD_BANK_FIXED_NL %d\n#define RBD_BANK_FIXED_L0 %d\n#define RBD_BANK_FIXED_PERM 0x%llxull\n#define RBD_BANK_FIXED_NS ", nlevels, L0, perm_down);
+  s += b;
+  for (int l = 0; l < nlevels; ++l) { snprintf(b, sizeof b, "%s%d", l ? "," : "", (int)nslots[l]); s += b; }
+}
+void bank_aba_entry(std::string& s, const char* tag, const char* T, const char* sfx, bool fused, const char* SI) {
+  char b[1600];
+  snprintf(b, sizeof b, "extern \"C\" __global__ __launch_bounds__(256, RBD_BANK_WAVES) void aba_bank_%sspec_%s(rbd::BankModel M, long B, const %s* q, const %s* v, const %s* tau,\n"
+                        "    const %s* fext, %s* vdot, %s* qdot, rbd::Layout Lq, rbd::Layout Lv, rbd::Layout Lf, rbd::MkFuse F) {\n",
+           tag, sfx, T, T, T, T, T, T);
+  s += b;
+  snprintf(b, sizeof b, "  __shared__ __align__(16) unsigned char lds[(size_t)rbd::BANK_LDS_PAIRS * 256 * sizeof(rbd::Pair2<%s>)];\n", T);
+  s += b;
+  snprintf(b, sizeof b, "  rbd::aba_bank_body<%s, %s, %s>(M, B, q, v, tau, fext, vdot, qdot, Lq, Lv, Lf, F, reinterpret_cast<rbd::Pair2<%s>*>(lds));\n}\n", T, fused ? "true" : "false", SI, T);
+  s += b;
+}
+}
 std::string spec_bank_source(int nlevels, int L0, const int32_t* nslots, unsigned long long perm_down, int simple, int dtype) {
   if (nlevels < 2 || nlevels > 64 || L0 < 1 || L0 >= nlevels) return std::string();
   const char* T = dtype == RBD_F32 ? "float" : "double";
@@ -551,27 +570,36 @@
   char b[1600];
   s += "// generated by rbd_jit.hip: the level structure of one mechanism for the banked kernels (aba_bank_body / rnea_bank_body, rbd_bank.hpp): loops over the levels unrolled,\n"
        "// DPP hop or exchange column and the number of later children known per level\n";
-  snprintf(b, sizeof b, "#define RBD_BANK_FIXED_NL %d\n#define RBD_BANK_FIXED_L0 %d\n#define RBD_BANK_FIXED_PERM 0x%llxull\n#define RBD_BANK_FIXED_NS ", nlevels, L0, perm_down);
-  s += b;
-  for (int l = 0; l < nlevels; ++l) { snprintf(b, sizeof b, "%s%d", l ? "," : "", (int)nslots[l]); s += b; }
+  bank_level_defines(s, nlevels, L0, nslots, perm_down);
   s += "\n#include \"rbd_lane.hpp\"\n#include \"rbd_bank.hpp\"\n";
-  const char* lds = "  __shared__ __align__(16) unsigned char lds[(size_t)rbd::BANK_LDS_PAIRS * 256 * sizeof(rbd::Pair2<%s>)];\n";
-  for (int fused = 0; fused < 2; ++fused) {
-    snprintf(b, sizeof b, "extern \"C\" __global__ __launch_bounds__(256, RBD_BANK_WAVES) void aba_bank_%sspec_%s(rbd::BankModel M, long B, const %s* q, const %s* v, const %s* tau,\n"
-                          "    const %s* fext, %s* vdot, %s* qdot, rbd::Layout Lq, rbd::Layout Lv, rbd::Layout Lf, rbd::MkFuse F) {\n",
-             fused ? "fused_" : "", sfx, T, T, T, T, T, T);
-    s += b;
-    snprintf(b, sizeof b, lds, T);
-    s += b;
-    snprintf(b, sizeof b, "  rbd::aba_bank_body<%s, %s, %s>(M, B, q, v, tau, fext, vdot, qdot, Lq, Lv, Lf, F, reinterpret_cast<rbd::Pair2<%s>*>(lds));\n}\n", T, fused ? "true" : "false", SI, T);
-    s += b;
-  }
+  for (int fused = 0; fused < 2; ++fused) bank_aba_entry(s, fused ? "fused_" : "", T, sfx, fused != 0, SI);
   snprintf(b, sizeof b, "extern \"C\" __global__ __launch_bounds__(256, 2) void rnea_bank_spec_%s(rbd::BankModel M, long B, int ncol, const %s* q, const %s* v, const %s* vdot, const %s* fext,\n"
                         "    %s* tau, %s* qdot, rbd::Layout Lq, rbd::Layout Lv, rbd::Layout Lf, %s* acc_out, %s* jw_out) {\n"
                         "  __shared__ __align__(16) unsigned char lds[(size_t)rbd::RNEA_LDS_PAIRS * 256 * sizeof(rbd::Pair2<%s>)];\n"
                         "  rbd::rnea_bank_body<%s, %s>(M, B, ncol, q, v, vdot, fext, tau, qdot, Lq, Lv, Lf, acc_out, jw_out, reinterpret_cast<rbd::Pair2<%s>*>(lds));\n}\n",
            sfx, T, T, T, T, T, T, T, T, T, T, SI, T);
   s += b;
+  return s;
+}
+std::string spec_bank_rr_source(const BankRrTables& R, int dtype) {
+  if (R.nlevels < 2 || R.nlevels > 64 || R.L0 < 1 || R.L0 >= R.nlevels || R.nchain < 1 || R.nchain > RC_MAX) return std::string();
+  const char* T = dtype == RBD_F32 ? "float" : "double";
+  const char* sfx = dtype == RBD_F32 ? "f32" : "f64";
+  std::string s;
+  char b[400];
+  s += "// generated by rbd_jit.hip: plain dynamics! of one floating-base mechanism on the tree re-rooted at its centre (rbd_reroot.hpp) for the banked kernel (aba_bank_body,\n"
+       "// rbd_bank.hpp): the re-rooted tree's level structure, and the chain of original joints from the old floating body to the new root as literals\n";
+  bank_level_defines(s, R.nlevels, R.L0, R.nslots, R.perm_down);
+  snprintf(b, sizeof b, "\n#define RBD_BANK_RR 1\n#define RBD_BANK_RR_NCHAIN %d\n#define RBD_BANK_RR_FQ %d\n#define RBD_BANK_RR_FV %d\n#define RBD_BANK_RR_FB_BANK %d\n#define RBD_BANK_RR_CHAIN_I ",
+           R.nchain, R.fq, R.fv, R.fb_bank);
+  s += b;
+  for (int k = 0; k < R.nchain * 4; ++k) { snprintf(b, sizeof b, "%s%d", k ? "," : "", (int)R.chain_i[k]); s += b; }
+  s += "\n#define RBD_BANK_RR_CHAIN_R ";
+  for (int k = 0; k < R.nchain * 15; ++k) { snprintf(b, sizeof b, "%s%.17g", k ? "," : "", R.chain_r[k]); s += b; }
+  s += "\n#define RBD_BANK_RR_FXP ";
+  for (int k = 0; k < 12; ++k) { snprintf(b, sizeof b, "%s%.17g", k ? "," : "", R.fXp[k]); s += b; }
+  s += "\n#include \"rbd_lane.hpp\"\n#include \"rbd_bank.hpp\"\n";
+  bank_aba_entry(s, "rr_", T, sfx, false, "true");
   return s;
 }
 
diff --git a/rigidbodydynamics.jl_amd/csrc/rbd_jit.hpp b/rigidbodydynamics.jl_amd/csrc/rbd_jit.hpp
--- a/rigidbodydynamics.jl_amd/csrc/rbd_jit.hpp
+++ b/rigidbodydynamics.jl_amd/csrc/rbd_jit.hpp
@@ -21,6 +21,15 @@
 };
 std::string spec_loop_source(const LoopTables& L, int dtype);
 std::string spec_bank_source(int nlevels, int L0, const int32_t* nslots, unsigned long long perm_down, int simple, int dtype);
+enum { SPEC_BANK_RR_FAMILY = 12 };
+struct BankRrTables {
+  int nlevels, L0, nchain, fq, fv, fb_bank;
+  const int32_t* nslots;
+  unsigned long long perm_down;
+  const int32_t* chain_i;
+  const double *chain_r, *fXp;
+};
+std::string spec_bank_rr_source(const BankRrTables& R, int dtype);
 struct WalkTables {
   int ns, G, nA, nB, nS, nq, nv, flt, gen, rr;
   const std::vector<int32_t>*ri, *wk;
diff --git a/rigidbodydynamics.jl_amd/state.py b/rigidbodydynamics.jl_amd/state.py
--- a/rigidbodydynamics.jl_amd/state.py
+++ b/rigidbodydynamics.jl_amd/state.py
@@ -846,7 +846,7 @@
     try:
         dt = _capi.F64 if dtype == torch.float64 else _capi.F32
         fam = {"mass_matrix": 0, "dynamics": 1, "inverse_dynamics": 2, "loops": 3, "dynamics_tracks": 4, "inverse_dynamics_tracks": 5, "dynamics_tracks_pairs": 6,
-               "inverse_dynamics_tracks_pairs": 7, "banked": 8, "dynamics_tracks_sim": 9, "dynamics_tracks_pairs_sim": 10, "kinematics": 11}[family]
+               "inverse_dynamics_tracks_pairs": 7, "banked": 8, "dynamics_tracks_sim": 9, "dynamics_tracks_pairs_sim": 10, "kinematics": 11, "banked_rerooted": 12}[family]
         n = L.rbd_jit_source(h, dt, fam, None, 0)
         if n < 0:
             return None
```

Result: slower. 214.1 million (-1.4%).
